# It4innovations/hyperqueue

Measured on AMD Instinct MI355X. Metric: tasks_assigned_per_sec, higher is better.
Workload: dtype u64

## Files before the change

hyperqueue_amd/csrc/debug_capi.cpp:

```cpp
#include "../../include/hqtick_debug.h"

#include "hb_order.h"
#include "milp.h"
#include "price_emul.h"

static thread_local int g_last_canonical = 0;
static thread_local long g_last_hull[2] = {0, 0};
extern "C" int hqtick_debug_milp_was_canonical(void) { return g_last_canonical; }
extern "C" void hqtick_debug_milp_last_hull(long *solves, long *nonpacking) {
    if (solves) *solves = g_last_hull[0];
    if (nonpacking) *nonpacking = g_last_hull[1];
}

extern "C" int hqtick_debug_milp_solve(int ncols, const double *obj, const uint8_t *col_kind, int nrows, const uint8_t *row_type,
                                       const double *rhs, const int *row_off, const int *row_col, const double *row_coef,
                                       double time_limit_s, int canonical, double *x_out, double *obj_out, int *is_optimal,
                                       long *nodes_out) {
    hqmilp::Model m;
    m.obj.assign(obj, obj + ncols);
    m.kind.assign(col_kind, col_kind + ncols);
    m.rtype.assign(row_type, row_type + nrows);
    m.rhs.assign(rhs, rhs + nrows);
    m.roff.assign(row_off, row_off + nrows + 1);
    int nnz = nrows ? row_off[nrows] : 0;
    m.rcol.assign(row_col, row_col + nnz);
    m.rcoef.assign(row_coef, row_coef + nnz);
    hqmilp::Result r = hqmilp::solve(m, time_limit_s, canonical != 0);
    g_last_canonical = r.canonical ? 1 : 0;
    g_last_hull[0] = r.hull_solves; g_last_hull[1] = r.hull_solves_nonpacking;
    if (nodes_out) *nodes_out = r.nodes;
    if (!r.feasible) return 0;
    for (int j = 0; j < ncols; j++) x_out[j] = r.x[j];
    *obj_out = r.objective;
    *is_optimal = r.optimal ? 1 : 0;
    return 1;
}

extern "C" void hqtick_debug_map_order_u32(const uint32_t *keys, uint32_t n, uint32_t *out_pos) {
    std::vector<uint32_t> order;
    hqhb::insertion_order_u32(keys, n, order);
    for (uint32_t i = 0; i < n; i++) out_pos[i] = order[i];
}

extern "C" int hqtick_debug_milp_solve_priced(int ncols, const double *obj, const uint8_t *col_kind, const int32_t *col_group, int nrows, const uint8_t *row_type,
                                              const uint8_t *row_implied, const double *rhs, const int *row_off, const int *row_col, const double *row_coef,
                                              double time_limit_s, int use_sweeps, uint32_t min_cols, double *x_out, double *obj_out, int *is_optimal, double *stats_out) {
    hqmilp::Model m;
    m.obj.assign(obj, obj + ncols);
    m.kind.assign(col_kind, col_kind + ncols);
    m.rtype.assign(row_type, row_type + nrows);
    m.rhs.assign(rhs, rhs + nrows);
    m.roff.assign(row_off, row_off + nrows + 1);
    int nnz = nrows ? row_off[nrows] : 0;
    m.rcol.assign(row_col, row_col + nnz);
    m.rcoef.assign(row_coef, row_coef + nnz);
    if (col_group) m.col_group.assign(col_group, col_group + ncols);
    if (row_implied) m.row_implied.assign(row_implied, row_implied + nrows);
    hqprice::EmulatedSweeper emu;
    if (min_cols) emu.min_cols = min_cols;
    hqmilp::Result r = hqmilp::solve(m, time_limit_s, true, hqmilp::REFERENCE_MIP_REL_GAP, use_sweeps ? &emu : nullptr);
    g_last_canonical = r.canonical ? 1 : 0;
    g_last_hull[0] = r.hull_solves; g_last_hull[1] = r.hull_solves_nonpacking;
    if (stats_out) { stats_out[0] = r.price_sweeps; stats_out[1] = r.price_rounds; stats_out[2] = r.price_total_us; stats_out[3] = r.canonical ? 1.0 : 0.0; }
    if (!r.feasible) return 0;
    for (int j = 0; j < ncols; j++) x_out[j] = r.x[j];
    *obj_out = r.objective;
    *is_optimal = r.optimal ? 1 : 0;
    return 1;
}

static thread_local hqmilp::Probe g_block_run_probe;
extern "C" void hqtick_debug_set_block_runs(int on) {
    hqmilp::g_probe = on < 0 ? nullptr : &g_block_run_probe; hqmilp::set_block_runs(on);
    if (on >= 0) { g_block_run_probe.model = g_block_run_probe.tables = g_block_run_probe.runs = g_block_run_probe.covered = 0; }
}
extern "C" void hqtick_debug_corrupt_block_runs(int on) { g_block_run_probe.corrupt_runs = on != 0; }
extern "C" void hqtick_debug_last_coupled_digest(uint64_t out[4]) {
    out[0] = g_block_run_probe.model; out[1] = g_block_run_probe.tables; out[2] = g_block_run_probe.runs; out[3] = g_block_run_probe.covered;
}
```

hyperqueue_amd/csrc/price.cpp:

```cpp
#include "price.h"

#include <algorithm>
#include <chrono>
#include <cmath>
#include <cstdio>
#include <cstring>
#include <functional>
#include <map>
#include <numeric>

#include "lp_tab.h"
#include "milp.h"

namespace hqprice {
namespace {

using hqmilp::lp::BASIC;
using hqmilp::lp::INF;
using hqmilp::lp::LP_OPT;
using hqmilp::lp::Rows;
using hqmilp::lp::Tab;

constexpr int KMAX_HOST = 128;
constexpr int NMAX_BLOCK = 32, MMAX_BLOCK = 4;
constexpr double FIRST_PROPOSAL_SCALE = 1.0 / 16.0;
constexpr double GRID = 10000.0;
constexpr int MAX_ROUNDS = 6;
constexpr int BP_MAX_NODES = 600;
constexpr double BP_MAX_STEPS = 3.0e6;
constexpr double BP_MAX_WORK = 3.0e9;

double now_us() { return std::chrono::duration<double, std::micro>(std::chrono::steady_clock::now().time_since_epoch()).count(); }

struct CapRow { int flat; double rhs; std::vector<std::pair<int, double>> g; };

struct Prob {
    HostTables T;
    std::vector<int> flat_of, model_of;
    std::vector<int> gmodel;
    std::vector<double> gcost;
    int K = 0, G = 0;
    std::vector<double> h;
    std::vector<uint8_t> ge;
    std::vector<std::vector<std::pair<int, double>>> g_rows;
    std::vector<int> grp_of;
    int KG = 0;
    std::vector<int> g_off, g_col; std::vector<int32_t> g_coef;
    std::vector<int> gr_off, gr_row;
    size_t row_terms = 0;
    std::vector<CapRow> caps;
    std::vector<int32_t> base_cap;
    std::vector<int> block_of_flat;
    int n_runs = 0, run_blocks = 0;
};

inline double round_fast(double v) { return (double)(long long)(v + (v >= 0.0 ? 0.5 : -0.5)); }
long long gcd_ll(long long a, long long b) { while (b) { const long long t = a % b; a = b; b = t; } return a < 0 ? -a : a; }

void finish_groups(Prob &P, const std::vector<std::vector<std::pair<int, int32_t>>> &lhs) {
    HostTables &T = P.T;
    const int KG = P.KG;
    T.K = (uint32_t)KG;
    size_t tot = 0; for (auto &l : lhs) tot += l.size();
    P.g_off.assign((size_t)KG + 1, 0); P.g_col.resize(tot); P.g_coef.resize(tot);
    std::vector<uint32_t> gcnt(T.n_cols + 1, 0);
    {
        auto *gc = P.g_col.data(); auto *gk = P.g_coef.data(); uint32_t *cnt = gcnt.data() + 1; size_t pos = 0;
        for (int g = 0; g < KG; g++) {
            const std::pair<int, int32_t> *l = lhs[(size_t)g].data();
            for (size_t i = 0, e = lhs[(size_t)g].size(); i < e; i++) { gc[pos] = l[i].first; gk[pos] = l[i].second; cnt[l[i].first]++; pos++; }
            P.g_off[(size_t)g + 1] = (int)pos;
        }
    }
    T.col_woff.assign(T.n_cols + 1, 0);
    for (uint32_t f = 0; f < T.n_cols; f++) T.col_woff[f + 1] = T.col_woff[f] + gcnt[f + 1];
    T.w_row.resize(T.col_woff[T.n_cols]); T.w_coef.resize(T.col_woff[T.n_cols]);
    {
        std::vector<uint32_t> &cur = gcnt;
        for (uint32_t f = 0; f < T.n_cols; f++) cur[f] = T.col_woff[f];
        uint32_t *cp = cur.data(); uint16_t *wr = T.w_row.data(); auto *wc = T.w_coef.data();
        const auto *gc = P.g_col.data(); const auto *gk = P.g_coef.data();
        for (int g = 0; g < KG; g++) for (int e = P.g_off[g], e1 = P.g_off[g + 1]; e < e1; e++) { const uint32_t p = cp[gc[e]]++; wr[p] = (uint16_t)g; wc[p] = gk[e]; }
    }
    P.gr_off.assign((size_t)KG + 1, 0);
    for (int k = 0; k < P.K; k++) P.gr_off[P.grp_of[k] + 1]++;
    for (int g = 0; g < KG; g++) P.gr_off[g + 1] += P.gr_off[g];
    P.gr_row.resize(P.K);
    { std::vector<int> c2(P.gr_off.begin(), P.gr_off.end() - 1); for (int k = 0; k < P.K; k++) P.gr_row[c2[P.grp_of[k]]++] = k; }
}

const char *build(const Request &rq, Prob &P) {
    const int n = rq.n;
    if (!rq.col_group) return "no block hints";
    std::vector<int> gid; gid.reserve(n);
    int max_group = -1;
    for (int j = 0; j < n; j++) max_group = std::max(max_group, rq.col_group[j]);
    std::vector<int> block_of_group((size_t)max_group + 1, -1);
    std::vector<int> bsize;
    std::vector<int> blk(n, -1);
    for (int j = 0; j < n; j++) {
        const int g = rq.col_group[j];
        if (g < 0) { P.gmodel.push_back(j); continue; }
        if (block_of_group[g] < 0) { block_of_group[g] = (int)bsize.size(); bsize.push_back(0); }
        blk[j] = block_of_group[g];
        if (++bsize[blk[j]] > NMAX_BLOCK) return "block with more than 32 columns";
    }
    const int nb = (int)bsize.size();
    if (nb < 8) return "fewer than 8 blocks";
    P.G = (int)P.gmodel.size();
    for (int j : P.gmodel) {
        if (rq.ub[j] != 1.0) return "global column that is not 0/1";
        if (rq.c[j] < 0.0) return "global column with negative cost";
        P.gcost.push_back(rq.c[j]);
    }
    std::vector<int> gidx(n, -1);
    for (int g = 0; g < P.G; g++) gidx[P.gmodel[g]] = g;
    HostTables &T = P.T;
    T.n_blocks = (uint32_t)nb;
    T.blk_off.assign((size_t)nb + 1, 0);
    for (int b = 0; b < nb; b++) T.blk_off[b + 1] = T.blk_off[b] + (uint32_t)bsize[b];
    T.n_cols = T.blk_off[nb];
    P.flat_of.assign(n, -1); P.model_of.assign(T.n_cols, -1); P.block_of_flat.assign(T.n_cols, -1);
    {
        std::vector<uint32_t> cur(T.blk_off.begin(), T.blk_off.end() - 1);
        for (int j = 0; j < n; j++) if (blk[j] >= 0) { const int f = (int)cur[blk[j]]++; P.flat_of[j] = f; P.model_of[f] = j; P.block_of_flat[f] = blk[j]; }
    }
    T.col_cost.assign(T.n_cols, 0.0); T.col_a.assign((size_t)T.n_cols * MMAX_BLOCK, 0.0); T.col_cap.assign(T.n_cols, 0);
    T.blk_m.assign(nb, 0); T.blk_cap.assign((size_t)nb * MMAX_BLOCK, 0.0);
    for (uint32_t f = 0; f < T.n_cols; f++) {
        const int j = P.model_of[f];
        if (rq.c[j] < 0.0) return "negative cost";
        if (!(rq.ub[j] <= 65535.0)) return "column bound above 65535";
        T.col_cost[f] = rq.c[j];
        T.col_cap[f] = (int32_t)std::floor(rq.ub[j] + 1e-9);
    }
    struct WideTmp { double h; uint8_t ge; std::vector<std::pair<int, int32_t>> cols; std::vector<std::pair<int, double>> g; };
    std::vector<WideTmp> wide;
    std::vector<std::pair<int, long long>> ai;
    for (int i = 0; i < rq.m; i++) {
        const int a = rq.roff[i], e = rq.roff[i + 1];
        if (a == e) continue;
        const double sc = rq.row_scale[i];
        int b0 = -2; bool multi = false, has_g = false, nonneg = true;
        int n_bcols = 0;
        for (int k = a; k < e; k++) {
            const int j = rq.rcol[k];
            if (rq.rcoef[k] < 0.0) nonneg = false;
            if (blk[j] < 0) { has_g = true; continue; }
            n_bcols++;
            if (b0 == -2) b0 = blk[j]; else if (blk[j] != b0) multi = true;
        }
        const bool is_le = rq.rlo[i] <= -INF, is_ge = rq.rhi[i] >= INF;
        if (is_le && is_ge) continue;
        if (!multi && !has_g && b0 >= 0) {
            if (rq.row_implied && rq.row_implied[i]) continue;
            if (is_le && nonneg) {
                double amax = 0.0;
                for (int k = a; k < e; k++) amax += rq.rcoef[k] * rq.ub[rq.rcol[k]];
                if (amax <= rq.rhi[i] * (1.0 + 1e-12) + 1e-9) continue;
            }
            if (!is_le || !nonneg || rq.rhi[i] < 0.0) return "block row that is not a packing row";
            const int r = T.blk_m[b0];
            if (r >= MMAX_BLOCK) {
                if (rq.trace) { fprintf(stderr, "[price] 5th row of block %d: hi %.6f scale %.6f:", b0, rq.rhi[i], sc); for (int k = a; k < e; k++) fprintf(stderr, " %.6f*x%d(ub %.0f)", rq.rcoef[k] * sc, rq.rcol[k], rq.ub[rq.rcol[k]]); fprintf(stderr, "\n"); }
                return "block with more than 4 rows";
            }
            long long g = 0; bool ok = true;
            ai.clear();
            for (int k = a; k < e && ok; k++) {
                const double v = rq.rcoef[k] * sc * GRID, rv = std::round(v);
                if (rv < 1.0 || std::fabs(v - rv) > 1e-6 * std::max(1.0, rv) || rv >= 4.0e15) ok = false;
                else { ai.push_back({P.flat_of[rq.rcol[k]], (long long)rv}); g = gcd_ll(g, (long long)rv); }
            }
            if (!ok) return "block row off the ResourceAmount grid";
            const double capv = rq.rhi[i] * sc * GRID;
            if (capv >= 4.0e15) return "block row capacity too large";
            const long long capi = (long long)std::floor(capv + 1e-6);
            if (g < 1) g = 1;
            for (auto &t : ai) T.col_a[(size_t)t.first * MMAX_BLOCK + r] += (double)(t.second / g);
            T.blk_cap[(size_t)b0 * MMAX_BLOCK + r] = (double)(capi / g);
            T.blk_m[b0] = (uint8_t)(r + 1);
            continue;
        }
        if (!is_le && !is_ge) return "equality or range row across blocks";
        if (is_le && nonneg) {
            double amax = 0.0;
            for (int k = a; k < e; k++) amax += rq.rcoef[k] * rq.ub[rq.rcol[k]];
            if (amax <= rq.rhi[i] * (1.0 + 1e-12) + 1e-9) continue;
        }
        if (is_ge && nonneg && rq.rlo[i] <= 1e-12) continue;
        if (!multi && has_g && n_bcols >= 1 && is_le && nonneg) {
            if (n_bcols != 1) return "conditional bound over several columns of a block";
            CapRow cr; cr.flat = -1; cr.rhs = 0.0;
            double cx = 0.0;
            for (int k = a; k < e; k++) if (blk[rq.rcol[k]] >= 0) { cr.flat = P.flat_of[rq.rcol[k]]; cx = rq.rcoef[k]; }
            if (!(cx > 0.0)) return "conditional bound with a zero coefficient";
            cr.rhs = rq.rhi[i] / cx;
            for (int k = a; k < e; k++) if (blk[rq.rcol[k]] < 0) cr.g.push_back({gidx[rq.rcol[k]], rq.rcoef[k] / cx});
            P.caps.push_back(std::move(cr));
            continue;
        }
        if (n_bcols == 0) return "row over global columns only";
        WideTmp w; w.ge = is_ge ? 1 : 0;
        w.cols.reserve((size_t)(e - a));
        const double sign = is_le ? 1.0 : -1.0;
        w.h = sign * (is_le ? rq.rhi[i] : rq.rlo[i]) * sc;
        for (int k = a; k < e; k++) {
            const int j = rq.rcol[k];
            const double v = sign * rq.rcoef[k] * sc;
            if (blk[j] < 0) { w.g.push_back({gidx[j], v}); continue; }
            const double rv = std::round(v);
            if (std::fabs(v - rv) > 1e-7 * std::max(1.0, std::fabs(rv)) || std::fabs(rv) > 1.0e9) return "wide row with a non-integer coefficient";
            if (rv != 0.0) w.cols.push_back({P.flat_of[j], (int32_t)rv});
        }
        wide.push_back(std::move(w));
        if ((int)wide.size() > 1024) return "more than 1024 wide rows";
    }
    for (int b = 0; b < nb; b++) if (T.blk_m[b] == 0) {
        double total = 0.0;
        for (uint32_t f = T.blk_off[b]; f < T.blk_off[b + 1]; f++) { T.col_a[(size_t)f * MMAX_BLOCK] = 1.0; total += (double)T.col_cap[f]; }
        T.blk_cap[(size_t)b * MMAX_BLOCK] = total;
        T.blk_m[b] = 1;
    }
    P.K = (int)wide.size();
    if (P.K == 0) return "no wide row";
    P.h.resize(P.K); P.ge.resize(P.K); P.g_rows.assign(P.G, {});
    std::vector<uint64_t> sig(P.K);
    for (int k = 0; k < P.K; k++) {
        P.h[k] = wide[k].h; P.ge[k] = wide[k].ge;
        uint64_t hsh = 1469598103934665603ull;
        for (auto &t : wide[k].cols) { hsh = (hsh ^ (uint64_t)(uint32_t)t.first) * 1099511628211ull; hsh = (hsh ^ (uint64_t)(uint32_t)t.second) * 1099511628211ull; }
        sig[k] = hsh; P.row_terms += wide[k].cols.size();
        for (auto &t : wide[k].g) P.g_rows[t.first].push_back({k, t.second});
    }
    P.grp_of.assign(P.K, -1);
    std::vector<int> rep;
    for (int k = 0; k < P.K; k++) {
        int g = -1;
        for (size_t i = 0; i < rep.size() && g < 0; i++) if (sig[rep[i]] == sig[k] && wide[rep[i]].cols == wide[k].cols) g = (int)i;
        if (g < 0) { g = (int)rep.size(); rep.push_back(k); }
        P.grp_of[k] = g;
    }
    P.KG = (int)rep.size();
    if (P.KG > KMAX_HOST) return "more than 128 distinct wide left-hand sides";
    std::vector<std::vector<std::pair<int, int32_t>>> lhs((size_t)P.KG);
    for (int g = 0; g < P.KG; g++) lhs[(size_t)g] = std::move(wide[rep[g]].cols);
    finish_groups(P, lhs);
    P.base_cap = T.col_cap;
    return nullptr;
}

struct Cut {
    double cx = 0, bnd = 0; std::vector<long long> act; std::vector<double> pi;
    std::vector<uint16_t> x; bool fetched = false; std::vector<std::pair<uint32_t, int32_t>> lo;
    std::vector<double> pcx; std::vector<long long> pact;
};

struct BPNode { std::vector<int8_t> flag; std::vector<std::pair<uint32_t, int32_t>> lo, hi; double bound = INF; int depth = 0; };

struct Solver {
    const Request &rq; Sweeper &sw; Prob P;
    std::vector<Cut> cuts;
    double relaxed_bound = INF;
    std::vector<double> relaxed_pi;
    double theta_scale = 1.0;
    std::vector<double> pmax;
    bool failed = false;
    size_t cut_lo = 0;
    double work = 0.0;
    double sweep_steps = 0.0; int budget_sweeps = 0;
    int max_sweeps = 256;
    std::vector<std::pair<uint32_t, int32_t>> node_lo, node_caps; double node_cl = 0.0; std::vector<double> node_Al; bool at_root = true;
    bool base_caps = true;
    Solver(const Request &r, Sweeper &s) : rq(r), sw(s) {}

    bool evaluate_launch(const std::vector<double> &pi) {
        if ((int)cuts.size() >= max_sweeps) return false;
        std::vector<double> pig(P.KG, 0.0);
        for (int k = 0; k < P.K; k++) pig[P.grp_of[k]] += pi[k];
        const double t0 = now_us();
        sw.pending_k = (uint32_t)P.KG;
        if (!sw.sweep_launch(pig.data())) { failed = true; return false; }
        sw.stat_sweep_us += now_us() - t0;
        return true;
    }
    int evaluate(const std::vector<double> &pi, bool launched = false) {
        if ((int)cuts.size() >= max_sweeps) return -1;
        SweepTotals tot;
        const double t0 = now_us();
        if (launched) { if (!sw.sweep_finish(tot)) { failed = true; return -1; } }
        else {
            std::vector<double> pig(P.KG, 0.0);
            for (int k = 0; k < P.K; k++) pig[P.grp_of[k]] += pi[k];
            if (!sw.sweep(pig.data(), tot)) { failed = true; return -1; }
        }
        sw.stat_sweep_us += now_us() - t0; sw.stat_sweeps++;
        if (!sw.merges_clock() && now_us() * 1e-6 > sw.guard_s) sw.time_up = true;
        sweep_steps += 64.0 + (double)tot.max_steps;
        if (tot.n_budget > std::max<uint32_t>(4, P.T.n_blocks / 64)) budget_sweeps++;
        Cut c; c.cx = tot.cx; c.bnd = tot.bnd; c.pi = pi;
        c.act.resize(P.K);
        for (int k = 0; k < P.K; k++) c.act[k] = tot.act[P.grp_of[k]];
        if (node_lo.empty() && tot.part_cx.size() == (size_t)PARTS && tot.part_act.size() == (size_t)PARTS * P.KG) {
            c.pcx = tot.part_cx; c.pact.resize((size_t)PARTS * P.K);
            for (int p = 0; p < PARTS; p++) for (int k = 0; k < P.K; k++) c.pact[(size_t)p * P.K + k] = tot.part_act[(size_t)p * P.KG + P.grp_of[k]];
        }
        if (!node_lo.empty()) {
            c.lo = node_lo; c.cx += node_cl; c.bnd += node_cl;
            for (int k = 0; k < P.K; k++) { c.act[k] += (long long)std::llround(node_Al[k]); c.bnd -= pi[k] * node_Al[k]; }
        }
        cuts.push_back(std::move(c));
        double L = cuts.back().bnd;
        for (int k = 0; k < P.K; k++) L += pi[k] * P.h[k];
        for (int g = 0; g < P.G; g++) { double r = P.gcost[g]; for (auto &t : P.g_rows[g]) r -= pi[t.first] * t.second; if (r > 0.0) L += r; }
        if (base_caps && at_root && L < relaxed_bound) { relaxed_bound = L; relaxed_pi = pi; }
        return (int)cuts.size() - 1;
    }
    double fixed_value(const Cut &c, const std::vector<double> &hB, double cB) const {
        double L = c.bnd + cB;
        for (int k = 0; k < P.K; k++) L += c.pi[k] * hB[k];
        return L;
    }

    bool aggregate_prices(const std::vector<double> &hB, const std::vector<int> &lk, std::vector<double> &pi) {
        const HostTables &T = P.T;
        static const int chunks_env = getenv("HQPRICE_AGG_CHUNKS") ? atoi(getenv("HQPRICE_AGG_CHUNKS")) : 0;
        uint32_t widest = 1;
        for (uint32_t b = 0; b < T.n_blocks; b++) widest = std::max(widest, T.blk_off[b + 1] - T.blk_off[b]);
        const int agg_chunks = chunks_env > 0 ? chunks_env : std::min(64, std::max(PARTS, (int)(256u / widest)));
        const uint32_t nb = T.n_blocks, per = (nb + (uint32_t)agg_chunks - 1) / (uint32_t)agg_chunks;
        const int NP = (int)((nb + per - 1) / per), KL = (int)lk.size();
        if (NP < 2 || KL == 0) return false;
        static const uint64_t min_cols_env = getenv("HQPRICE_AGG_MINCOLS") ? (uint64_t)atoll(getenv("HQPRICE_AGG_MINCOLS")) : 32768;
        if ((uint64_t)T.n_cols < min_cols_env) return false;
        if (P.G != 0) return false;
        std::vector<uint32_t> pb0(NP), pcnt(NP), pnc(NP), voff(NP + 1, 0);
        for (int p = 0; p < NP; p++) {
            const uint32_t b0 = (uint32_t)p * per, b1 = std::min(nb, b0 + per);
            pb0[p] = b0; pcnt[p] = b1 - b0; pnc[p] = T.blk_off[b0 + 1] - T.blk_off[b0];
            const uint32_t c0 = T.blk_off[b0], nc = pnc[p];
            for (uint32_t b = b0 + 1; b < b1; b++) {
                const uint32_t c = T.blk_off[b];
                if (T.blk_off[b + 1] - c != nc || T.blk_m[b] != T.blk_m[b0]) return false;
                if (memcmp(&T.blk_cap[(size_t)b * MMAX_BLOCK], &T.blk_cap[(size_t)b0 * MMAX_BLOCK], sizeof(double) * MMAX_BLOCK) != 0) return false;
                if (memcmp(&T.col_a[(size_t)c * MMAX_BLOCK], &T.col_a[(size_t)c0 * MMAX_BLOCK], sizeof(double) * MMAX_BLOCK * nc) != 0) return false;
                if (memcmp(&T.col_cap[c], &T.col_cap[c0], sizeof(int32_t) * nc) != 0) return false;
                for (uint32_t q = 0; q < nc; q++) {
                    const uint32_t e0 = T.col_woff[c0 + q], e1 = T.col_woff[c0 + q + 1], f0 = T.col_woff[c + q];
                    if (T.col_woff[c + q + 1] - f0 != e1 - e0) return false;
                    if (e1 > e0 && (memcmp(&T.w_row[f0], &T.w_row[e0], sizeof(uint16_t) * (e1 - e0)) != 0 || memcmp(&T.w_coef[f0], &T.w_coef[e0], sizeof(int32_t) * (e1 - e0)) != 0)) return false;
                }
            }
            voff[p + 1] = voff[p] + nc;
        }
        const int nv = (int)voff[NP];
        if (nv == 0 || nv > 8192) return false;
        Rows A; A.n = nv;
        std::vector<double> ac(nv), alb(nv, 0.0), aub(nv);
        std::vector<std::pair<int, double>> terms;
        for (int p = 0; p < NP; p++) {
            const uint32_t c0 = T.blk_off[pb0[p]], nc = pnc[p];
            for (uint32_t q = 0; q < nc; q++) {
                double sum = 0.0;
                for (uint32_t b = 0; b < pcnt[p]; b++) sum += T.col_cost[T.blk_off[pb0[p] + b] + q];
                ac[voff[p] + q] = sum / (double)pcnt[p] / theta_scale;
                aub[voff[p] + q] = (double)pcnt[p] * (double)T.col_cap[c0 + q];
            }
            for (int r = 0; r < (int)T.blk_m[pb0[p]]; r++) {
                terms.clear(); double sc = 0.0;
                for (uint32_t q = 0; q < nc; q++) { const double a = T.col_a[(size_t)(c0 + q) * MMAX_BLOCK + r]; if (a != 0.0) { terms.push_back({(int)(voff[p] + q), a}); sc = std::max(sc, std::fabs(a)); } }
                if (terms.empty()) continue;
                for (auto &t : terms) t.second /= sc;
                A.add(terms, -INF, (double)pcnt[p] * T.blk_cap[(size_t)pb0[p] * MMAX_BLOCK + r] / sc);
            }
        }
        const int first_wide = A.m;
        std::vector<double> wscale(KL, 1.0);
        for (int i = 0; i < KL; i++) {
            const int g = P.grp_of[lk[i]];
            terms.clear(); double sc = 0.0;
            for (int p = 0; p < NP; p++) {
                const uint32_t c0 = T.blk_off[pb0[p]];
                for (uint32_t q = 0; q < pnc[p]; q++) for (uint32_t e = T.col_woff[c0 + q]; e < T.col_woff[c0 + q + 1]; e++) if ((int)T.w_row[e] == g) { terms.push_back({(int)(voff[p] + q), (double)T.w_coef[e]}); sc = std::max(sc, std::fabs((double)T.w_coef[e])); }
            }
            if (terms.empty()) { A.add({{0, 0.0}}, -INF, INF); continue; }
            for (auto &t : terms) t.second /= sc;
            wscale[i] = sc;
            A.add(terms, -INF, hB[lk[i]] / sc);
        }
        Tab at; at.init(&A, ac, alb, aub);
        if (at.solve(20000) != LP_OPT) return false;
        work += at.ops;
        pi.assign(P.K, 0.0);
        bool any = false;
        for (int i = 0; i < KL; i++) {
            const int a = at.where[first_wide + i];
            if (a < 0 || at.st[A.n + a] == BASIC) continue;
            double y = std::fabs(at.d[A.n + a]) / wscale[i] * theta_scale;
            if (!(y > 0.0)) continue;
            pi[lk[i]] = std::min(y, pmax[lk[i]]);
            any = true;
        }
        return any;
    }

    std::function<bool(const std::vector<double> &, double)> probe;
    struct Settled { bool valid = false; std::vector<double> hB, lambda, pi; double cB = 0.0, bound = 0.0; size_t n_cuts = 0, cut_lo = 0; } settled;
    bool kelley(const std::vector<double> &hB, double cB, double cutoff, double tol, std::vector<double> &lambda, std::vector<double> &pi_out, double *bound_out, bool no_sweeps = false) {
        if (!no_sweeps && settled.valid) {
            settled.valid = false;
            if (settled.n_cuts == cuts.size() && settled.cut_lo == cut_lo && settled.cB == cB && settled.hB == hB) {
                if (settled.bound < cutoff) return false;
                lambda = std::move(settled.lambda); pi_out = std::move(settled.pi); *bound_out = settled.bound;
                return true;
            }
        }
        const int K = P.K;
        const uint32_t per = (P.T.n_blocks + PARTS - 1) / PARTS;
        const int NP = (int)((P.T.n_blocks + per - 1) / per);
        std::vector<int> lk; lk.reserve(P.KG);
        for (int g = 0; g < P.KG; g++) {
            int best = -1;
            for (int q = P.gr_off[g]; q < P.gr_off[g + 1]; q++) { const int k = P.gr_row[q]; if (best < 0 || hB[k] < hB[best]) best = k; }
            if (best >= 0) lk.push_back(best);
        }
        std::sort(lk.begin(), lk.end());
        const int KL = (int)lk.size();
        Rows M; M.n = KL + NP;
        std::vector<double> mc(KL + NP), mlb(KL + NP, 0.0), mub(KL + NP);
        for (int i = 0; i < KL; i++) { mc[i] = -hB[lk[i]] / theta_scale; mub[i] = pmax[lk[i]]; }
        for (int p = 0; p < NP; p++) { mc[KL + p] = -1.0; mub[KL + p] = 4.0; }
        std::vector<double> cut_scale;
        std::vector<std::pair<int, double>> terms;
        size_t in_master = cut_lo;
        auto push_cuts = [&](Tab *mt) {
            for (; in_master < cuts.size(); in_master++) {
                const Cut &c = cuts[in_master];
                for (int p = 0; p < NP; p++) {
                    terms.clear(); double sc = 1.0;
                    for (int i = 0; i < KL; i++) { const long long a = c.pact[(size_t)p * K + lk[i]]; if (a != 0) { const double v = (double)a / theta_scale; terms.push_back({i, v}); sc = std::max(sc, std::fabs(v)); } }
                    terms.push_back({KL + p, 1.0});
                    for (auto &t : terms) t.second /= sc;
                    M.add(terms, c.pcx[p] / theta_scale / sc, INF);
                    cut_scale.push_back(sc);
                    if (mt) mt->where.push_back(-1);
                }
            }
        };
        for (size_t k = cut_lo; k < cuts.size(); k++) if (cuts[k].pcx.empty()) { if (rq.trace) fprintf(stderr, "[price] master: cut %zu without part sums\n", k); return false; }
        push_cuts(nullptr);
        Tab mt; mt.init(&M, mc, mlb, mub);
        double ub_best = INF; std::vector<double> pi_best(K, 0.0);
        for (size_t k = cut_lo; k < cuts.size(); k++) { const double L = fixed_value(cuts[k], hB, cB); if (L < ub_best) { ub_best = L; pi_best = cuts[k].pi; } }
        std::vector<double> pi(K, 0.0), pi_prev_master;
        double lb_master = -INF, lp_us = 0.0;
        bool converged = false; int probes = 0;
        auto multipliers = [&](std::vector<double> &lambda) {
            lambda.assign(cuts.size() * PARTS, 0.0);
            std::vector<double> lsum(NP, 0.0);
            for (size_t r = 0; r / NP + cut_lo < cuts.size() && r < (size_t)M.m; r++) {
                const int a = mt.where[r];
                if (a < 0 || mt.st[M.n + a] == BASIC) continue;
                const size_t k = r / NP + cut_lo; const int p = (int)(r % NP);
                const double v = std::fabs(mt.d[M.n + a]) / cut_scale[r];
                lambda[k * PARTS + p] = v; lsum[p] += v;
            }
            for (int p = 0; p < NP; p++) if (!(lsum[p] > 0.0)) {
                size_t bk = cut_lo; double bv = -INF;
                for (size_t k = cut_lo; k < cuts.size(); k++) {
                    double v = cuts[k].pcx[p];
                    for (int i = 0; i < KL; i++) v -= mt.x[i] * (double)cuts[k].pact[(size_t)p * K + lk[i]];
                    if (v > bv) { bv = v; bk = k; }
                }
                lambda[bk * PARTS + p] = 1.0; lsum[p] = 1.0;
            }
            for (size_t k = cut_lo; k < cuts.size(); k++) for (int p = 0; p < NP; p++) lambda[k * PARTS + p] /= lsum[p];
        };
        for (int it = 0; it < 200; it++) {
            { const double tl0 = now_us(); const int st = mt.solve(200000); lp_us += now_us() - tl0; if (st != LP_OPT) { if (rq.trace) fprintf(stderr, "[price] master LP status %d at iteration %d (%d cuts)\n", st, it, M.m); return false; } }
            lb_master = -mt.objective() * theta_scale + cB;
            if (ub_best < cutoff) { if (rq.trace) fprintf(stderr, "[price] configuration bounded by %.9f, below the incumbent %.9f\n", ub_best, cutoff); return false; }
            if (ub_best - lb_master <= tol * std::fabs(ub_best)) { converged = true; break; }
            if (no_sweeps) return false;
            if (probe && probes < 3 && it >= 1 && ub_best - lb_master <= 0.1 * std::fabs(ub_best)) {
                probes++;
                std::vector<double> lam, colact(K, 0.0);
                multipliers(lam);
                for (size_t k = cut_lo; k < cuts.size(); k++) for (int p = 0; p < NP; p++) {
                    const double l = lam[k * PARTS + p];
                    if (l == 0.0) continue;
                    const long long *pa = &cuts[k].pact[(size_t)p * K];
                    for (int r = 0; r < K; r++) colact[r] += l * (double)pa[r];
                }
                auto keep = std::move(probe); probe = nullptr;
                const bool go = keep(colact, lb_master);
                probe = std::move(keep);
                if (go) return false;
            }
            bool same = !pi_prev_master.empty();
            for (int i = 0; i < KL && same; i++) same = std::fabs(mt.x[i] - pi_prev_master[i]) <= 1e-15 + 1e-12 * std::fabs(mt.x[i]);
            pi_prev_master.assign(mt.x.begin(), mt.x.begin() + KL);
            const double alpha = (it < 3 || same) ? 0.0 : 0.3;
            for (int k = 0; k < K; k++) pi[k] = alpha * pi_best[k];
            for (int i = 0; i < KL; i++) pi[lk[i]] += (1.0 - alpha) * mt.x[i];
            if (it == 0 && cut_lo == 0 && cuts.size() == 1) {
                std::vector<double> pa;
                static const bool agg_on = !(getenv("HQPRICE_AGG_START") && atoi(getenv("HQPRICE_AGG_START")) == 0);
                if (agg_on && aggregate_prices(hB, lk, pa)) { pi = pa; if (rq.trace) fprintf(stderr, "[price]   first proposal: the duals of the model aggregated over chunks of blocks\n"); }
                else for (int k = 0; k < K; k++) pi[k] *= FIRST_PROPOSAL_SCALE;
            }
            const int ci = evaluate(pi);
            if (ci < 0) break;
            if (sw.time_up) { if (rq.trace) fprintf(stderr, "[price] 70 %% of the time limit gone inside the master loop\n"); return false; }
            if (budget_sweeps >= 8) { if (rq.trace) fprintf(stderr, "[price] blocks keep running out of their search budget (%d sweeps): not a model for the sweeps\n", budget_sweeps); return false; }
            const double L = fixed_value(cuts[ci], hB, cB);
            if (L < ub_best) { ub_best = L; pi_best = pi; }
            push_cuts(&mt);
        }
        if (!converged) {
            if (mt.solve(200000) != LP_OPT) return false;
            lb_master = -mt.objective() * theta_scale + cB;
            if (ub_best - lb_master > 1e-3 * std::fabs(ub_best)) { if (rq.trace) fprintf(stderr, "[price] master not converged: %.9f vs %.9f\n", ub_best, lb_master); return false; }
        }
        multipliers(lambda);
        if (rq.trace) fprintf(stderr, "[price]   master: %d priced rows + %d parts, %d cut rows, %ld pivots, %.1f us inside the LP (%d active rows)\n", KL, NP, M.m, mt.iters, lp_us, mt.ma);
        pi_out.assign(K, 0.0);
        for (int i = 0; i < KL; i++) pi_out[lk[i]] = mt.x[i];
        *bound_out = ub_best;
        if (no_sweeps) { settled.valid = true; settled.hB = hB; settled.cB = cB; settled.lambda = lambda; settled.pi = pi_out; settled.bound = ub_best; settled.n_cuts = cuts.size(); settled.cut_lo = cut_lo; }
        return true;
    }

    bool fetch_patterns() {
        size_t first = cuts.size();
        for (size_t k = 0; k < cuts.size(); k++) if (!cuts[k].fetched) { first = k; break; }
        if (first == cuts.size()) return true;
        const uint32_t count = (uint32_t)(cuts.size() - first);
        const uint16_t *pat = sw.patterns((uint32_t)first, count);
        if (!pat) { failed = true; return false; }
        const uint32_t nc = P.T.n_cols;
        for (uint32_t i = 0; i < count; i++) {
            Cut &c = cuts[first + i];
            if (c.fetched) continue;
            c.x.assign(pat + (size_t)i * nc, pat + (size_t)(i + 1) * nc);
            for (auto &l : c.lo) c.x[l.first] = (uint16_t)(c.x[l.first] + l.second);
            c.fetched = true;
        }
        return true;
    }

    std::vector<uint16_t> round_patterns(const std::vector<double> &lambda, const std::vector<double> &pi, const std::vector<double> &hB,
                                         const std::vector<char> *usable = nullptr, const std::vector<int32_t> *lo_of = nullptr, int variant = 0) {
        const int K = P.K; const HostTables &T = P.T;
        const uint32_t S = (uint32_t)cuts.size();
        const double t_r0 = now_us();
        if (!fetch_patterns()) return {};
        auto pat_of = [&](int k) { return cuts[(size_t)k].x.data(); };
        const uint32_t per = (T.n_blocks + PARTS - 1) / PARTS;
        auto lam = [&](int k, uint32_t p) { return lambda[(size_t)k * PARTS + p]; };
        std::vector<int> active;
        for (uint32_t k = 0; k < S; k++) {
            if (usable && !(*usable)[k]) continue;
            bool any = false; for (uint32_t p = 0; p < (uint32_t)PARTS && !any; p++) any = lam((int)k, p) > 1e-9;
            if (any) active.push_back((int)k);
        }
        if (active.empty()) return {};
        const int Q = (int)active.size();
        std::vector<double> lpact(K, 0.0), wgt(K);
        for (int k : active) {
            const Cut &c = cuts[k];
            if (c.pact.empty()) { for (int r = 0; r < K; r++) lpact[r] += lam(k, 0) * (double)c.act[r]; continue; }
            for (uint32_t p = 0; p < (uint32_t)PARTS; p++) { const double l = lam(k, p); if (l > 0.0) for (int r = 0; r < K; r++) lpact[r] += l * (double)c.pact[(size_t)p * P.K + r]; }
        }
        for (int r = 0; r < K; r++) {
            const bool tight = pi[r] > 1e-12 || hB[r] - lpact[r] <= 1e-6 * std::max(1.0, std::fabs(hB[r]));
            wgt[r] = (tight ? 1.0 : 0.02) / std::max(1.0, std::fabs(hB[r]));
        }
        auto block_act = [&](uint32_t b, const uint16_t *x, std::vector<double> &out) {
            double ga[KMAX_HOST];
            for (int g = 0; g < P.KG; g++) ga[g] = 0.0;
            for (uint32_t f = T.blk_off[b]; f < T.blk_off[b + 1]; f++) { const uint16_t xv = x[f]; if (!xv) continue; for (uint32_t e = T.col_woff[f]; e < T.col_woff[f + 1]; e++) ga[T.w_row[e]] += (double)T.w_coef[e] * (double)xv; }
            for (int r = 0; r < K; r++) out[r] = ga[P.grp_of[r]];
        };
        std::vector<uint16_t> x(T.n_cols, 0);
        std::vector<double> cum(K, 0.0);
        std::vector<int> chosen(T.n_blocks, 0);
        {
            const int KG = P.KG;
            std::vector<double> wg(KG, 0.0), cumg(KG, 0.0), tgtg(KG, 0.0), candg((size_t)Q * KG);
            for (int r = 0; r < K; r++) wg[P.grp_of[r]] += wgt[r];
            std::vector<char> on(Q); std::vector<const double *> cgp(Q, nullptr);
            for (uint32_t bi = 0; bi < T.n_blocks; bi++) {
                const uint32_t b = variant == 1 ? T.n_blocks - 1 - bi : bi;
                const uint32_t part = b / per;
                int first = -1; bool all_same = true;
                const size_t blk_bytes = (size_t)(T.blk_off[b + 1] - T.blk_off[b]) * 2;
                for (int q = 0; q < Q; q++) {
                    const double l = lam(active[q], part);
                    on[q] = l > 1e-9;
                    if (!on[q]) continue;
                    const uint16_t *px = pat_of(active[q]);
                    if (first >= 0 && memcmp(px + T.blk_off[b], pat_of(active[first]) + T.blk_off[b], blk_bytes) == 0) cgp[q] = cgp[first];
                    else {
                        if (first < 0) first = q; else all_same = false;
                        double *cg = &candg[(size_t)q * KG];
                        for (int g = 0; g < KG; g++) cg[g] = 0.0;
                        for (uint32_t f = T.blk_off[b]; f < T.blk_off[b + 1]; f++) { const uint16_t xv = px[f]; if (!xv) continue; for (uint32_t e = T.col_woff[f]; e < T.col_woff[f + 1]; e++) cg[T.w_row[e]] += (double)T.w_coef[e] * (double)xv; }
                        cgp[q] = cg;
                    }
                    const double *cg = cgp[q];
                    for (int g = 0; g < KG; g++) tgtg[g] += l * cg[g];
                }
                int bq = -1; double be = INF;
                if (all_same) bq = first;
                else for (int q = 0; q < Q; q++) {
                    if (!on[q]) continue;
                    const double *cg = cgp[q];
                    double e = 0.0;
                    for (int g = 0; g < KG; g++) e += std::fabs(cumg[g] + cg[g] - tgtg[g]) * wg[g];
                    if (e < be - 1e-15) { be = e; bq = q; }
                }
                if (bq < 0) return {};
                const double *cb = cgp[bq];
                for (int g = 0; g < KG; g++) cumg[g] += cb[g];
                chosen[b] = active[bq];
                memcpy(&x[T.blk_off[b]], pat_of(active[bq]) + T.blk_off[b], (size_t)(T.blk_off[b + 1] - T.blk_off[b]) * 2);
            }
            for (int r = 0; r < K; r++) cum[r] = cumg[P.grp_of[r]];
        }
        if (rq.trace) fprintf(stderr, "[price]   rounding: diffusion done at %.3f us, %d active cuts\n", now_us() - t_r0, Q);
        auto ge_short = [&](const std::vector<double> &c) { double s = 0.0; for (int r = 0; r < K; r++) if (P.ge[r] && c[r] > hB[r] + 1e-9) s += c[r] - hB[r]; return s; };
        if (ge_short(cum) > 0.0) {
            std::vector<int> pool = active;
            for (int k = (int)S - 1; k >= 0 && (int)pool.size() < Q + 12; k--) if ((!usable || (*usable)[k]) && std::find(pool.begin(), pool.end(), k) == pool.end()) pool.push_back(k);
            std::vector<double> a0(K), a1(K), c2(K);
            double cmax = 0.0; for (double c : T.col_cost) cmax = std::max(cmax, c);
            struct Cand { double score; uint32_t b; int k; };
            std::vector<Cand> cl; std::vector<double> colshort, coltight;
            auto evaluate_switch = [&](uint32_t b, int k, double v0, double &score) {
                const uint16_t *px = pat_of(k);
                block_act(b, px, a1);
                double gain = 0.0, newviol = 0.0;
                for (int r = 0; r < K; r++) {
                    if (a0[r] == a1[r]) continue;
                    const double c = cum[r] - a0[r] + a1[r];
                    if (P.ge[r]) gain += std::max(0.0, cum[r] - hB[r]) - std::max(0.0, c - hB[r]);
                    else newviol += std::max(0.0, c - hB[r]) - std::max(0.0, cum[r] - hB[r]);
                }
                if (!(gain > 1e-9)) return false;
                double v1 = 0.0; for (uint32_t f = T.blk_off[b]; f < T.blk_off[b + 1]; f++) v1 += T.col_cost[f] * (double)px[f];
                score = gain * 10.0 * cmax - (v0 - v1) - std::max(0.0, newviol) * cmax;
                return true;
            };
            auto value_of = [&](uint32_t b) { double v = 0.0; for (uint32_t f = T.blk_off[b]; f < T.blk_off[b + 1]; f++) v += T.col_cost[f] * (double)x[f]; return v; };
            for (int pass = 0; pass < 64 && ge_short(cum) > 0.0; pass++) {
                const double base = ge_short(cum);
                cl.clear();
                std::vector<int> short_in(P.KG, 0);
                for (int r = 0; r < K; r++) if (P.ge[r] && cum[r] > hB[r] + 1e-9) short_in[P.grp_of[r]]++;
                std::vector<int> tight_in(P.KG, 0);
                double spare = 0.0;
                for (int r = 0; r < K; r++) if (P.ge[r] && cum[r] <= hB[r] + 1e-9 && hB[r] - cum[r] <= 2.0 + 1e-9) { tight_in[P.grp_of[r]]++; spare += std::max(0.0, hB[r] - cum[r]); }
                colshort.assign(T.n_cols, 0.0); coltight.assign(T.n_cols, 0.0);
                for (uint32_t f = 0; f < T.n_cols; f++) for (uint32_t e = T.col_woff[f]; e < T.col_woff[f + 1]; e++) {
                    const int ns = short_in[T.w_row[e]], nt = tight_in[T.w_row[e]];
                    if (ns) colshort[f] += (double)ns * (double)T.w_coef[e];
                    if (nt) coltight[f] += (double)nt * (double)T.w_coef[e];
                }
                for (uint32_t b = 0; b < T.n_blocks; b++) {
                    for (int k : pool) {
                        if (k == chosen[b]) continue;
                        const uint16_t *px = pat_of(k);
                        double gain = 0.0, dv = 0.0, dmg = 0.0; bool differs = false;
                        for (uint32_t f = T.blk_off[b]; f < T.blk_off[b + 1]; f++) {
                            const int d = (int)px[f] - (int)x[f];
                            if (!d) continue;
                            differs = true; dv += T.col_cost[f] * (double)d;
                            gain -= colshort[f] * (double)d;
                            dmg += coltight[f] * (double)d;
                        }
                        if (!differs || !(gain - std::max(0.0, dmg - spare) > 1e-9)) continue;
                        cl.push_back({std::min(gain, base) * 10.0 * cmax + dv, b, k});
                    }
                }
                if (rq.trace) fprintf(stderr, "[price]     pass %d: short by %.1f, %zu candidate switches, at %.3f us\n", pass, base, cl.size(), now_us() - t_r0);
                if (cl.empty()) break;
                const size_t top = std::min<size_t>(cl.size(), 512);
                std::partial_sort(cl.begin(), cl.begin() + (long)top, cl.end(), [](const Cand &p, const Cand &q) { return p.score > q.score || (p.score == q.score && (p.b < q.b || (p.b == q.b && p.k < q.k))); });
                cl.resize(top);
                std::vector<char> moved(T.n_blocks, 0);
                for (const Cand &cd : cl) {
                    if (!(ge_short(cum) > 0.0)) break;
                    if (moved[cd.b]) continue;
                    {
                        const uint16_t *px = pat_of(cd.k); double gain = 0.0;
                        for (uint32_t f = T.blk_off[cd.b]; f < T.blk_off[cd.b + 1]; f++) {
                            const int d = (int)px[f] - (int)x[f];
                            if (d) for (uint32_t e = T.col_woff[f]; e < T.col_woff[f + 1]; e++) { const int g = T.w_row[e]; for (int q = P.gr_off[g]; q < P.gr_off[g + 1]; q++) { const int r = P.gr_row[q]; if (P.ge[r] && cum[r] > hB[r] + 1e-9) gain -= (double)T.w_coef[e] * (double)d; } }
                        }
                        if (!(gain > 1e-9)) continue;
                    }
                    block_act(cd.b, pat_of(chosen[cd.b]), a0);
                    double score;
                    if (!evaluate_switch(cd.b, cd.k, value_of(cd.b), score)) continue;
                    for (int r = 0; r < K; r++) cum[r] += a1[r] - a0[r];
                    chosen[cd.b] = cd.k; moved[cd.b] = 1;
                    memcpy(&x[T.blk_off[cd.b]], pat_of(cd.k) + T.blk_off[cd.b], (size_t)(T.blk_off[cd.b + 1] - T.blk_off[cd.b]) * 2);
                }
                if (ge_short(cum) >= base - 1e-9) break;
            }
            if (ge_short(cum) > 0.0) return {};
        }
        if (rq.trace) fprintf(stderr, "[price]   rounding: >= repair done at %.3f us\n", now_us() - t_r0);
        for (int r = 0; r < K; r++) {
            if (cum[r] <= hB[r] + 1e-9) continue;
            std::vector<int> cols;
            const int gr = P.grp_of[r];
            for (int k = P.g_off[gr]; k < P.g_off[gr + 1]; k++) if (P.g_coef[k] > 0 && x[P.g_col[k]] > 0) cols.push_back(k);
            std::sort(cols.begin(), cols.end(), [&](int a, int b) { const double ca = T.col_cost[P.g_col[a]] / P.g_coef[a], cb = T.col_cost[P.g_col[b]] / P.g_coef[b]; return ca < cb || (ca == cb && a > b); });
            for (int k : cols) {
                const int f = P.g_col[k];
                while (x[f] > (lo_of ? (uint16_t)(*lo_of)[f] : 0) && cum[r] > hB[r] + 1e-9) {
                    bool ok = true;
                    for (uint32_t e = T.col_woff[f]; e < T.col_woff[f + 1] && ok; e++) if (T.w_coef[e] < 0) { const int g = T.w_row[e]; for (int q = P.gr_off[g]; q < P.gr_off[g + 1] && ok; q++) if (cum[P.gr_row[q]] - (double)T.w_coef[e] > hB[P.gr_row[q]] + 1e-9) ok = false; }
                    if (!ok) break;
                    x[f]--;
                    for (uint32_t e = T.col_woff[f]; e < T.col_woff[f + 1]; e++) { const int g = T.w_row[e]; for (int q = P.gr_off[g]; q < P.gr_off[g + 1]; q++) cum[P.gr_row[q]] -= (double)T.w_coef[e]; }
                }
                if (cum[r] <= hB[r] + 1e-9) break;
            }
            if (cum[r] > hB[r] + 1e-9) return {};
        }
        return x;
    }

    struct NodeLP { double bound = INF; bool pruned = false; std::vector<double> lambda, pi, bfrac; };

    bool apply_node(const BPNode &nd, std::vector<int32_t> &lo_arr, std::vector<int32_t> &hi_arr) {
        const HostTables &T = P.T;
        lo_arr.assign(T.n_cols, 0); hi_arr = P.base_cap;
        for (auto &l : nd.lo) lo_arr[l.first] = std::max(lo_arr[l.first], l.second);
        for (auto &h : nd.hi) hi_arr[h.first] = std::min(hi_arr[h.first], h.second);
        node_caps.clear();
        for (const CapRow &cr : P.caps) {
            double r = cr.rhs; bool all_fixed = true;
            for (auto &t : cr.g) { if (nd.flag[t.first] < 0) { all_fixed = false; break; } r -= t.second * (double)nd.flag[t.first]; }
            if (!all_fixed) continue;
            const double c = std::floor(r + 1e-9);
            const int32_t cap = c < 0.0 ? 0 : (c > 65535.0 ? 65535 : (int32_t)c);
            if (cap < hi_arr[cr.flat]) { hi_arr[cr.flat] = cap; node_caps.push_back({(uint32_t)cr.flat, cap}); }
        }
        std::vector<int32_t> caps(T.n_cols); std::vector<double> bcap(T.blk_cap);
        node_lo.clear(); node_cl = 0.0; node_Al.assign(P.K, 0.0);
        for (uint32_t f = 0; f < T.n_cols; f++) {
            if (hi_arr[f] < lo_arr[f]) return false;
            caps[f] = hi_arr[f] - lo_arr[f];
            const int32_t l = lo_arr[f];
            if (l <= 0) continue;
            node_lo.push_back({f, l}); node_cl += T.col_cost[f] * (double)l;
            for (uint32_t e = T.col_woff[f]; e < T.col_woff[f + 1]; e++) { const int g = T.w_row[e]; for (int q = P.gr_off[g]; q < P.gr_off[g + 1]; q++) node_Al[P.gr_row[q]] += (double)T.w_coef[e] * (double)l; }
            const int b = P.block_of_flat[f];
            for (int r = 0; r < MMAX_BLOCK; r++) bcap[(size_t)b * MMAX_BLOCK + r] -= T.col_a[(size_t)f * MMAX_BLOCK + r] * (double)l;
        }
        for (double v : bcap) if (v < 0.0) return false;
        if (!sw.set_caps(caps.data()) || !sw.set_block_caps(bcap.data())) { failed = true; return false; }
        at_root = nd.lo.empty() && nd.hi.empty() && node_caps.empty();
        return true;
    }

    void node_master(const BPNode &nd, double cutoff, double tol, NodeLP &out, std::vector<char> &usable) {
        const int K = P.K, G = P.G;
        out = NodeLP(); out.bound = nd.bound;
        if (!fetch_patterns()) return;
        usable.assign(cuts.size(), 1);
        for (size_t k = 0; k < cuts.size(); k++) {
            const std::vector<uint16_t> &x = cuts[k].x;
            for (auto &l : nd.lo) if ((int32_t)x[l.first] < l.second) { usable[k] = 0; break; }
            if (usable[k]) for (auto &h : nd.hi) if ((int32_t)x[h.first] > h.second) { usable[k] = 0; break; }
            if (usable[k]) for (auto &h : node_caps) if ((int32_t)x[h.first] > h.second) { usable[k] = 0; break; }
        }
        std::vector<double> hN(P.h); double cN = 0.0;
        std::vector<int> freeg;
        for (int g = 0; g < G; g++) {
            if (nd.flag[g] < 0) { freeg.push_back(g); continue; }
            cN += P.gcost[g] * (double)nd.flag[g];
            for (auto &t : P.g_rows[g]) hN[t.first] -= t.second * (double)nd.flag[g];
        }
        const int F = (int)freeg.size();
        Rows M; M.n = K + 1 + F;
        std::vector<double> mc(M.n), mlb(M.n, 0.0), mub(M.n);
        for (int k = 0; k < K; k++) { mc[k] = -hN[k] / theta_scale; mub[k] = pmax[k]; }
        mc[K] = -1.0; mub[K] = 4.0;
        for (int i = 0; i < F; i++) { mc[K + 1 + i] = -1.0; mub[K + 1 + i] = 4.0; }
        std::vector<std::pair<int, double>> terms;
        std::vector<double> row_scale; std::vector<int> row_cut;
        for (int i = 0; i < F; i++) {
            const int g = freeg[i];
            terms.clear(); double sc = 1.0;
            for (auto &t : P.g_rows[g]) { const double v = t.second / theta_scale; terms.push_back({t.first, v}); sc = std::max(sc, std::fabs(v)); }
            terms.push_back({K + 1 + i, 1.0});
            for (auto &t : terms) t.second /= sc;
            M.add(terms, P.gcost[g] / theta_scale / sc, INF);
            row_scale.push_back(sc); row_cut.push_back(-1);
        }
        Tab mt;
        auto add_cut = [&](size_t k, bool live) {
            const Cut &c = cuts[k];
            terms.clear(); double sc = 1.0;
            for (int r = 0; r < K; r++) if (c.act[r] != 0) { const double v = (double)c.act[r] / theta_scale; terms.push_back({r, v}); sc = std::max(sc, std::fabs(v)); }
            terms.push_back({K, 1.0});
            for (auto &t : terms) t.second /= sc;
            M.add(terms, c.cx / theta_scale / sc, INF);
            row_scale.push_back(sc); row_cut.push_back((int)k);
            if (live) mt.where.push_back(-1);
        };
        for (size_t k = 0; k < cuts.size(); k++) if (usable[k]) add_cut(k, false);
        mt.init(&M, mc, mlb, mub);
        auto node_value = [&](const Cut &c) {
            double L = c.bnd + cN;
            for (int k = 0; k < K; k++) L += c.pi[k] * hN[k];
            for (int g : freeg) { double r = P.gcost[g]; for (auto &t : P.g_rows[g]) r -= c.pi[t.first] * t.second; if (r > 0.0) L += r; }
            return L;
        };
        std::vector<double> pi(K), pi_best, prev;
        bool ok = false;
        for (int it = 0; it < 80; it++) {
            ok = false;
            if (mt.solve(200000) != LP_OPT) break;
            ok = true;
            const double lbm = -mt.objective() * theta_scale + cN;
            if (out.bound <= cutoff) { out.pruned = true; break; }
            if (out.bound - lbm <= tol * std::fabs(out.bound)) break;
            bool same = !prev.empty();
            for (int k = 0; k < K && same; k++) same = std::fabs(mt.x[k] - prev[k]) <= 1e-15 + 1e-12 * std::fabs(mt.x[k]);
            prev.assign(mt.x.begin(), mt.x.begin() + K);
            const double alpha = (it < 2 || same || pi_best.empty()) ? 0.0 : 0.3;
            for (int k = 0; k < K; k++) pi[k] = (alpha > 0.0 ? alpha * pi_best[k] : 0.0) + (1.0 - alpha) * mt.x[k];
            const int ci = evaluate(pi);
            if (ci < 0) { ok = false; break; }
            usable.push_back(1);
            const double L = node_value(cuts[ci]);
            if (L < out.bound) { out.bound = L; pi_best = pi; }
            add_cut((size_t)ci, true);
        }
        work += mt.ops;
        if (!ok || out.pruned) return;
        out.lambda.assign(cuts.size(), 0.0); out.bfrac.assign(G, 0.0);
        double lsum = 0.0;
        for (int r = 0; r < M.m; r++) {
            const int a = mt.where[r];
            if (a < 0 || mt.st[M.n + a] == BASIC) continue;
            const double v = std::fabs(mt.d[M.n + a]) / row_scale[r];
            if (row_cut[r] >= 0) { out.lambda[row_cut[r]] = v; lsum += v; } else out.bfrac[freeg[r]] = std::min(1.0, v);
        }
        for (int g = 0; g < G; g++) if (nd.flag[g] >= 0) out.bfrac[g] = (double)nd.flag[g];
        if (lsum > 0.0) for (double &l : out.lambda) l /= lsum; else out.lambda.clear();
        out.pi.assign(mt.x.begin(), mt.x.begin() + K);
    }
};

}

namespace {
Answer run_solver(Solver &S, const double tp0) {
    Answer ans;
    const Request &rq = S.rq; Sweeper &sw = S.sw;
    auto tmark = [&](const char *what) { if (rq.trace) fprintf(stderr, "[price] %s at %.3f ms (sweeps so far %.3f ms)\n", what, (now_us() - tp0) / 1e3, sw.stat_sweep_us / 1e3); };
    tmark("model flattened");
    if (rq.trace) fprintf(stderr, "[price]   %d equal-block runs took %d of %u blocks from their first one\n", S.P.n_runs, S.P.run_blocks, S.P.T.n_blocks);
    Prob &P = S.P;
    if (rq.trace) fprintf(stderr, "[price] %u blocks, %u block columns, %d wide rows with %d distinct left-hand sides (%zu / %zu terms), %d flags, %zu conditional bounds\n", P.T.n_blocks, P.T.n_cols, P.K, P.KG, P.row_terms, P.T.w_row.size(), P.G, P.caps.size());
    const int K = P.K, G = P.G;
    sw.stat_sweeps = 0; sw.stat_sweep_us = 0;
    sw.guard_s = rq.deadline_s - 0.3 * rq.time_limit_s; sw.time_up = false;
    S.max_sweeps = (int)std::min<size_t>(4096, std::max<size_t>(256, ((size_t)64 << 20) / ((size_t)P.T.n_cols * 2 + 1)));
    if (!sw.begin(P.T, (uint32_t)S.max_sweeps)) { ans.why = "sweeper refused the model"; return ans; }
    struct Ender { Sweeper &s; ~Ender() { s.end(); } } ender{sw};
    tmark("tables handed to the sweeper");
    std::vector<double> pi0(K, 0.0);
    if (!S.evaluate_launch(pi0)) { ans.why = "sweep failed"; return ans; }
    S.pmax.assign(K, 0.0);
    {
        double cmax = 0.0; for (double c : P.T.col_cost) cmax = std::max(cmax, c);
        std::vector<double> gp(P.KG, 0.0);
        for (int g = 0; g < P.KG; g++) {
            double p = 0.0; bool neg = false; int32_t amin = INT32_MAX;
            for (int t = P.g_off[g]; t < P.g_off[g + 1]; t++) {
                const int32_t a = P.g_coef[t];
                if (a > 0) p = std::max(p, P.T.col_cost[P.g_col[t]] / (double)a); else { neg = true; amin = std::min(amin, -a); }
            }
            if (neg) p = std::max(p, 64.0 * cmax / (double)std::max<int32_t>(1, amin));
            gp[g] = p;
        }
        for (int k = 0; k < K; k++) S.pmax[k] = gp[P.grp_of[k]];
    }
    tmark("price caps done");
    if (S.evaluate(pi0, true) < 0) { ans.why = "sweep failed"; return ans; }
    tmark("first sweep (prices 0) done");
    S.theta_scale = std::max(S.cuts[0].bnd, 1e-9);
    ans.ran = true;
    double best_value = rq.incumbent ? rq.incumbent_value : -INF;
    std::vector<double> hB(K);
    std::vector<int32_t> caps(P.base_cap);
    std::vector<double> final_pi;
    std::vector<std::vector<double>> tried;
    auto was_tried = [&](const std::vector<double> &B) { for (auto &t : tried) if (t == B) return true; return false; };
    auto certified = [&]() { return best_value > -INF && S.relaxed_bound <= best_value + rq.rel_gap * std::fabs(best_value); };
    std::vector<double> jump_to;
    auto try_config = [&](const std::vector<double> &B, std::vector<double> &x) -> double {
        tried.push_back(B);
        if (!sw.merges_clock() && now_us() * 1e-6 > sw.guard_s) sw.time_up = true;
        if (sw.time_up) return -INF;
        ans.rounds++;
        double cB = 0.0;
        for (int k = 0; k < K; k++) hB[k] = P.h[k];
        for (int g = 0; g < G; g++) { cB += P.gcost[g] * B[g]; for (auto &t : P.g_rows[g]) hB[t.first] -= t.second * B[g]; }
        if (!P.caps.empty()) {
            caps = P.base_cap;
            for (const CapRow &cr : P.caps) { double r = cr.rhs; for (auto &t : cr.g) r -= t.second * B[t.first]; const double c = std::floor(r + 1e-9); if (c < (double)caps[cr.flat]) caps[cr.flat] = c < 0.0 ? 0 : (int32_t)c; }
            if (!sw.set_caps(caps.data())) { S.failed = true; return -INF; }
            S.base_caps = false; S.cut_lo = S.cuts.size();
            if (S.evaluate(pi0) < 0) return -INF;
        }
        std::vector<double> lambda, pi;
        double bound_B = INF;
        const double cutoff = best_value > -INF ? best_value * (1.0 - 1e-12) : -INF;
        const double tol = std::max(1e-6, rq.rel_gap / 50.0);
        jump_to.clear();
        S.probe = nullptr;
        if (G > 0 && P.caps.empty()) S.probe = [&](const std::vector<double> &colact, double lb_here) -> bool {
            std::vector<double> Bp = B, act = colact;
            for (int g = 0; g < G; g++) if (Bp[g] == 1.0) for (auto &t : P.g_rows[g]) act[t.first] += t.second;
            bool dropped = false;
            for (int g = 0; g < G; g++) {
                if (Bp[g] != 1.0 || P.gcost[g] != 0.0) continue;
                bool ok = true;
                for (auto &t : P.g_rows[g]) if (act[t.first] - t.second > P.h[t.first] + 1e-7 * (1.0 + std::fabs(P.h[t.first]))) ok = false;
                if (!ok) continue;
                Bp[g] = 0.0; dropped = true;
                for (auto &t : P.g_rows[g]) act[t.first] -= t.second;
            }
            if (!dropped || was_tried(Bp)) return false;
            std::vector<double> hBp(K); double cBp = 0.0;
            for (int k = 0; k < K; k++) hBp[k] = P.h[k];
            for (int g = 0; g < G; g++) { cBp += P.gcost[g] * Bp[g]; for (auto &t : P.g_rows[g]) hBp[t.first] -= t.second * Bp[g]; }
            std::vector<double> lam2, pi2; double b2 = INF;
            if (!S.kelley(hBp, cBp, -INF, tol, lam2, pi2, &b2, true) || b2 < lb_here) { S.settled.valid = false; return false; }
            if (rq.trace) fprintf(stderr, "[price] configuration %u left for the one its fractional point names: converged on the %zu cuts at hand, bound %.9f\n", ans.rounds, S.cuts.size(), b2);
            jump_to = Bp;
            return true;
        };
        const bool conv = S.kelley(hB, cB, cutoff, tol, lambda, pi, &bound_B);
        S.probe = nullptr;
        if (!conv) return -INF;
        tmark("master converged");
        final_pi = pi;
        std::vector<uint16_t> xf = S.round_patterns(lambda, pi, hB);
        tmark("patterns rounded");
        if (xf.empty()) return -INF;
        x.assign(rq.n, 0.0);
        for (uint32_t f = 0; f < P.T.n_cols; f++) x[P.model_of[f]] = (double)xf[f];
        for (int g = 0; g < G; g++) x[P.gmodel[g]] = B[g];
        double value = 0.0;
        if (!rq.polish || !rq.polish(x, value)) return -INF;
        tmark("polished");
        if (rq.trace) fprintf(stderr, "[price] configuration %u: %zu sweeps so far, bound with these flags %.9f, point %.9f, model bound %.9f\n", ans.rounds, S.cuts.size(), bound_B, value, S.relaxed_bound);
        if (value > best_value) { best_value = value; ans.x = x; ans.x_value = value; }
        if (bound_B > best_value * (1.0 + rq.rel_gap)) {
            std::vector<uint16_t> xr = S.round_patterns(lambda, pi, hB, nullptr, nullptr, 1);
            if (!xr.empty()) {
                std::vector<double> x2(rq.n, 0.0);
                for (uint32_t f = 0; f < P.T.n_cols; f++) x2[P.model_of[f]] = (double)xr[f];
                for (int g = 0; g < G; g++) x2[P.gmodel[g]] = B[g];
                double v2 = 0.0;
                if (rq.polish(x2, v2)) {
                    if (rq.trace) fprintf(stderr, "[price] configuration %u, blocks in reverse order: point %.9f\n", ans.rounds, v2);
                    if (v2 > value) { value = v2; x = x2; }
                    if (v2 > best_value) { best_value = v2; ans.x = x2; ans.x_value = v2; }
                }
            }
        }
        return value;
    };
    auto drop_flags = [&](std::vector<double> &B, const std::vector<double> &x) {
        bool dropped = false;
        std::vector<double> act(K, 0.0);
        {
            std::vector<double> ga(P.KG, 0.0);
            for (int g = 0; g < P.KG; g++) for (int t = P.g_off[g]; t < P.g_off[g + 1]; t++) ga[g] += (double)P.g_coef[t] * x[P.model_of[P.g_col[t]]];
            for (int k = 0; k < K; k++) act[k] += ga[P.grp_of[k]];
        }
        for (int g = 0; g < G; g++) for (auto &t : P.g_rows[g]) act[t.first] += t.second * x[P.gmodel[g]];
        for (int g = 0; g < G; g++) {
            if (B[g] != 1.0 || P.gcost[g] != 0.0 || x[P.gmodel[g]] != 1.0) continue;
            bool ok = true;
            for (auto &t : P.g_rows[g]) if (act[t.first] - t.second > P.h[t.first] + 1e-7 * (1.0 + std::fabs(P.h[t.first]))) ok = false;
            if (!ok) continue;
            B[g] = 0.0; dropped = true;
            for (auto &t : P.g_rows[g]) act[t.first] -= t.second;
        }
        return dropped;
    };
    auto descend = [&](std::vector<double> B) {
        for (int round = 0; round < MAX_ROUNDS && !S.failed && !was_tried(B); round++) {
            std::vector<double> x;
            const double v = try_config(B, x);
            if (!jump_to.empty()) { B = jump_to; jump_to.clear(); continue; }
            if (v == -INF) break;
            if (certified()) break;
            if (!drop_flags(B, x)) break;
        }
    };
    if (rq.incumbent && G > 0) {
        std::vector<double> B(G);
        for (int g = 0; g < G; g++) B[g] = rq.incumbent[P.gmodel[g]] > 0.5 ? 1.0 : 0.0;
        descend(B);
    }
    if (ans.x.empty() && !S.failed) descend(std::vector<double>(G, 1.0));
    if (S.failed) { ans.ran = false; ans.why = "sweep failed"; ans.x.clear(); return ans; }
    std::vector<double> Blp;
    if (G > 0 && best_value > -INF && !certified()) {
        if (!S.base_caps) {
            if (!sw.set_caps(P.base_cap.data())) { ans.ran = false; ans.why = "sweep failed"; ans.x.clear(); return ans; }
            S.base_caps = true; S.cut_lo = S.cuts.size();
            if (S.evaluate(pi0) < 0) { ans.ran = false; ans.why = "sweep failed"; ans.x.clear(); return ans; }
        }
        Rows M; M.n = K + 1 + G;
        std::vector<double> mc(M.n), mlb(M.n, 0.0), mub(M.n);
        for (int k = 0; k < K; k++) { mc[k] = -P.h[k] / S.theta_scale; mub[k] = S.pmax[k]; }
        mc[K] = -1.0; mub[K] = 4.0;
        for (int g = 0; g < G; g++) { mc[K + 1 + g] = -1.0; mub[K + 1 + g] = 4.0; }
        std::vector<std::pair<int, double>> terms;
        for (int g = 0; g < G; g++) {
            terms.clear(); double sc = 1.0;
            for (auto &t : P.g_rows[g]) { const double v = t.second / S.theta_scale; terms.push_back({t.first, v}); sc = std::max(sc, std::fabs(v)); }
            terms.push_back({K + 1 + g, 1.0});
            for (auto &t : terms) t.second /= sc;
            M.add(terms, P.gcost[g] / S.theta_scale / sc, INF);
        }
        size_t in_master = S.cut_lo;
        Tab mt;
        auto push_cuts = [&](bool live) {
            for (; in_master < S.cuts.size(); in_master++) {
                const Cut &c = S.cuts[in_master];
                terms.clear(); double sc = 1.0;
                for (int k = 0; k < K; k++) if (c.act[k] != 0) { const double v = (double)c.act[k] / S.theta_scale; terms.push_back({k, v}); sc = std::max(sc, std::fabs(v)); }
                terms.push_back({K, 1.0});
                for (auto &t : terms) t.second /= sc;
                M.add(terms, c.cx / S.theta_scale / sc, INF);
                if (live) mt.where.push_back(-1);
            }
        };
        push_cuts(false);
        mt.init(&M, mc, mlb, mub);
        std::vector<double> pi(K), pi_best = S.relaxed_pi.empty() ? std::vector<double>(K, 0.0) : S.relaxed_pi, prev;
        bool master_ok = false;
        for (int it = 0; it < 120; it++) {
            master_ok = false;
            if (mt.solve(200000) != LP_OPT) break;
            master_ok = true;
            const double lb_master = -mt.objective() * S.theta_scale;
            if (S.relaxed_bound <= best_value + rq.rel_gap * std::fabs(best_value)) break;
            if (S.relaxed_bound - lb_master <= 1e-6 * std::fabs(S.relaxed_bound)) break;
            bool same = !prev.empty();
            for (int k = 0; k < K && same; k++) same = std::fabs(mt.x[k] - prev[k]) <= 1e-15 + 1e-12 * std::fabs(mt.x[k]);
            prev.assign(mt.x.begin(), mt.x.begin() + K);
            const double alpha = (it < 2 || same) ? 0.0 : 0.3;
            for (int k = 0; k < K; k++) pi[k] = alpha * pi_best[k] + (1.0 - alpha) * mt.x[k];
            const double before = S.relaxed_bound;
            if (S.evaluate(pi) < 0) break;
            if (S.relaxed_bound < before) pi_best = pi;
            push_cuts(true);
        }
        if (S.failed) { ans.ran = false; ans.why = "sweep failed"; ans.x.clear(); return ans; }
        if (master_ok || mt.solve(200000) == LP_OPT) {
            Blp.assign(G, 0.0);
            for (int g = 0; g < G; g++) { const int ar = mt.where[g]; if (ar >= 0 && mt.st[M.n + ar] != BASIC) { double sc = 1.0; for (auto &t : P.g_rows[g]) sc = std::max(sc, std::fabs(t.second / S.theta_scale)); Blp[g] = std::min(1.0, std::fabs(mt.d[M.n + ar]) / sc); } }
        }
    }
    if (!Blp.empty() && !certified() && P.caps.empty()) {
        std::vector<double> B(G);
        for (int g = 0; g < G; g++) B[g] = (Blp[g] > 0.5 || P.gcost[g] > 0.0) ? 1.0 : 0.0;
        descend(B);
        for (int trial = 0; trial < 12 && !certified() && !S.failed && !ans.x.empty(); trial++) {
            std::vector<double> cur(G);
            for (int g = 0; g < G; g++) cur[g] = ans.x[P.gmodel[g]];
            int pick = -1; double pv = INF;
            for (int g = 0; g < G; g++) {
                if (cur[g] != 1.0 || P.gcost[g] != 0.0) continue;
                std::vector<double> t = cur; t[g] = 0.0;
                if (was_tried(t)) continue;
                if (Blp[g] < pv) { pv = Blp[g]; pick = g; }
            }
            if (pick < 0) break;
            cur[pick] = 0.0;
            descend(cur);
        }
        if (S.failed) { ans.ran = false; ans.why = "sweep failed"; ans.x.clear(); return ans; }
    }
    double bp_bound = INF;
    if (best_value > -INF && !certified() && !S.failed && P.T.n_cols <= 131072 && S.budget_sweeps < 8) {
        S.base_caps = true;
        int col_nodes = 0;
        auto closes = [&](double bound) { return bound <= best_value + rq.rel_gap * std::fabs(best_value); };
        std::vector<BPNode> stack;
        { BPNode root; root.flag.assign(G, -1); root.bound = S.relaxed_bound; stack.push_back(std::move(root)); }
        double closed_max = -INF;
        int nodes = 0;
        std::vector<int32_t> lo_arr, hi_arr; std::vector<char> usable;
        while (!stack.empty() && nodes < BP_MAX_NODES && (int)S.cuts.size() + 8 < S.max_sweeps && S.work < BP_MAX_WORK * rq.time_limit_s && S.sweep_steps < BP_MAX_STEPS * rq.time_limit_s &&
               !sw.time_up && !S.failed) {
            BPNode nd = std::move(stack.back()); stack.pop_back();
            if (!sw.merges_clock() && now_us() * 1e-6 > sw.guard_s) { sw.time_up = true; stack.push_back(std::move(nd)); break; }
            if (closes(nd.bound)) { closed_max = std::max(closed_max, nd.bound); continue; }
            nodes++;
            if (!S.apply_node(nd, lo_arr, hi_arr)) { if (S.failed) break; continue; }
            Solver::NodeLP lp;
            S.node_master(nd, best_value, std::max(2e-6, rq.rel_gap / 20.0), lp, usable);
            if (S.failed) break;
            if (lp.pruned || closes(lp.bound)) { closed_max = std::max(closed_max, std::min(lp.bound, nd.bound)); continue; }
            if (lp.lambda.empty()) { stack.push_back(std::move(nd)); break; }
            nd.bound = std::min(nd.bound, lp.bound);
            int bg = -1; double bd = 1e-6;
            for (int g = 0; g < G; g++) if (nd.flag[g] < 0) { const double d = std::min(lp.bfrac[g], 1.0 - lp.bfrac[g]); if (d > bd) { bd = d; bg = g; } }
            if (bg < 0) {
                std::vector<double> Bn(G), hBn(P.h);
                for (int g = 0; g < G; g++) { Bn[g] = lp.bfrac[g] > 0.5 ? 1.0 : 0.0; for (auto &t : P.g_rows[g]) hBn[t.first] -= t.second * Bn[g]; }
                std::vector<double> lam_parts(lp.lambda.size() * PARTS);
                for (size_t k = 0; k < lp.lambda.size(); k++) for (int p = 0; p < PARTS; p++) lam_parts[k * PARTS + p] = lp.lambda[k];
                std::vector<uint16_t> xf = S.round_patterns(lam_parts, lp.pi, hBn, &usable, &lo_arr);
                if (!xf.empty()) {
                    std::vector<double> x(rq.n, 0.0);
                    for (uint32_t f = 0; f < P.T.n_cols; f++) x[P.model_of[f]] = (double)xf[f];
                    for (int g = 0; g < G; g++) x[P.gmodel[g]] = Bn[g];
                    double value = 0.0;
                    if (rq.polish && rq.polish(x, value) && value > best_value) { best_value = value; ans.x = x; ans.x_value = value; }
                }
                if (closes(nd.bound)) { closed_max = std::max(closed_max, nd.bound); continue; }
            }
            BPNode a = nd, b = nd; a.depth = b.depth = nd.depth + 1;
            if (bg >= 0) {
                const int8_t first = lp.bfrac[bg] > 0.5 ? 1 : 0;
                a.flag[bg] = first; b.flag[bg] = (int8_t)(1 - first);
            } else {
                if (++col_nodes > 48) { stack.push_back(std::move(nd)); break; }
                int bf = -1; double bs = 1e-7, bv = 0.0;
                std::vector<double> xl(P.T.n_cols, 0.0);
                for (size_t k = 0; k < S.cuts.size(); k++) { const double l = k < lp.lambda.size() ? lp.lambda[k] : 0.0; if (l <= 0.0 || !usable[k]) continue; const uint16_t *px = S.cuts[k].x.data(); for (uint32_t f = 0; f < P.T.n_cols; f++) xl[f] += l * (double)px[f]; }
                for (uint32_t f = 0; f < P.T.n_cols; f++) { const double fr = xl[f] - std::floor(xl[f]); const double sc = std::min(fr, 1.0 - fr) * (P.T.col_cost[f] + 1e-9); if (std::min(fr, 1.0 - fr) > 1e-6 && sc > bs) { bs = sc; bf = (int)f; bv = xl[f]; } }
                if (bf < 0) { closed_max = std::max(closed_max, nd.bound); continue; }
                const int32_t fl = (int32_t)std::floor(bv);
                BPNode dn = nd, up = nd; dn.depth = up.depth = nd.depth + 1;
                dn.hi.push_back({(uint32_t)bf, fl}); up.lo.push_back({(uint32_t)bf, fl + 1});
                if (bv - fl < 0.5) { a = std::move(dn); b = std::move(up); } else { a = std::move(up); b = std::move(dn); }
            }
            stack.push_back(std::move(b)); stack.push_back(std::move(a));
        }
        bp_bound = closed_max;
        for (const BPNode &nd : stack) bp_bound = std::max(bp_bound, nd.bound);
        if (rq.trace) fprintf(stderr, "[price] branch and price: %d nodes, %zu left open, %zu sweeps in all, bound %.9f, incumbent %.9f\n", nodes, stack.size(), S.cuts.size(), bp_bound, best_value);
        S.node_lo.clear(); S.at_root = true;
        if (S.failed) { ans.ran = false; ans.why = "sweep failed"; ans.x.clear(); return ans; }
    }
    ans.bound = std::min(S.relaxed_bound, bp_bound > -INF ? bp_bound : INF);
    ans.sweeps = (uint32_t)sw.stat_sweeps;
    const bool closed = best_value > -INF && ans.bound <= best_value + rq.rel_gap * std::fabs(best_value);
    if (!final_pi.empty() && !closed) {
        ans.block_of.assign(rq.n, -1); ans.rcost.assign(rq.n, 0.0);
        std::vector<std::pair<int, double>> rows;
        for (uint32_t f = 0; f < P.T.n_cols; f++) {
            const int j = P.model_of[f];
            ans.block_of[j] = P.block_of_flat[f];
            double r = P.T.col_cost[f];
            rows.clear();
            for (uint32_t e = P.T.col_woff[f]; e < P.T.col_woff[f + 1]; e++) { const int g = P.T.w_row[e]; for (int q = P.gr_off[g]; q < P.gr_off[g + 1]; q++) rows.push_back({P.gr_row[q], (double)P.T.w_coef[e]}); }
            std::sort(rows.begin(), rows.end());
            for (auto &t : rows) r -= final_pi[t.first] * t.second;
            ans.rcost[j] = r;
        }
    }
    return ans;
}
}

namespace {

thread_local bool g_check_hints = false; thread_local int g_hint_mismatches = 0;
const char *flatten_model(const ModelView &mv, Prob &P, std::vector<double> &ub, std::vector<double> &c, double &cmax) {
    const int n = mv.n, m = mv.m;
    if (!mv.col_group || !mv.row_lhs || !mv.row_lhs_len) return "no structure hints";
    int max_group = -1;
    for (int j = 0; j < n; j++) max_group = std::max(max_group, mv.col_group[j]);
    std::vector<int> block_of_group((size_t)max_group + 1, -1), bsize, blk(n, -1);
    for (int j = 0; j < n; j++) {
        const int g = mv.col_group[j];
        if (g < 0) { P.gmodel.push_back(j); continue; }
        if (block_of_group[g] < 0) { block_of_group[g] = (int)bsize.size(); bsize.push_back(0); }
        blk[j] = block_of_group[g];
        if (++bsize[blk[j]] > NMAX_BLOCK) return "block with more than 32 columns";
    }
    const int nb = (int)bsize.size();
    if (nb < 8) return "fewer than 8 blocks";
    cmax = 0.0;
    for (int j = 0; j < n; j++) cmax = std::max(cmax, std::fabs(mv.obj[j]));
    if (cmax == 0.0) cmax = 1.0;
    c.resize(n);
    for (int j = 0; j < n; j++) c[j] = mv.obj[j] / cmax;
    P.G = (int)P.gmodel.size();
    for (int j : P.gmodel) {
        if (mv.kind[j] != 1) return "global column that is not 0/1";
        if (c[j] < 0.0) return "global column with negative cost";
        P.gcost.push_back(c[j]);
    }
    std::vector<int> gidx(n, -1);
    for (int g = 0; g < P.G; g++) gidx[P.gmodel[g]] = g;
    const int n_lhs = mv.n_lists;
    for (int i = 0; i < m; i++) if (mv.row_lhs[i] >= n_lhs) return "bad structure hint";
    struct Fam { int first = -1, len = 0; bool has_neg = false, scanned = false; double rhs_min = INF;
                 int b0 = -2; bool multi = false, has_g = false, integral = true; int n_bcols = 0; double amax = 0.0; };
    std::vector<Fam> fam((size_t)n_lhs);
    ub.assign(n, INF);
    for (int j = 0; j < n; j++) if (mv.kind[j] == 1) ub[j] = 1.0;
    const bool hinted = mv.row_block && mv.col_ub;
    if (hinted) for (int j = 0; j < n; j++) if (mv.col_ub[j] != UINT32_MAX) ub[j] = std::min(ub[j], (double)mv.col_ub[j]);
    auto bound_terms = [&](int a, int e, double rhs) { for (int k = a; k < e; k++) if (mv.rcoef[k] > 0.0) { double &u = ub[mv.rcol[k]]; u = std::min(u, std::floor(rhs / mv.rcoef[k] + 1e-9)); } };
    for (int l = 0; l < n_lhs; l++) for (int k = mv.list_off[l]; k < mv.list_off[l + 1]; k++) if (mv.list_col[k] < 0 || mv.list_col[k] >= n) return "bad structure hint";
    for (int i = 0; i < m; i++) {
        const int a = mv.roff[i], e = mv.roff[i + 1];
        if (a == e && mv.row_lhs[i] < 0) { const double b = mv.rhs[i]; const bool ok = mv.rtype[i] == 1 ? b >= -1e-9 : (mv.rtype[i] == 0 ? b <= 1e-9 : std::fabs(b) <= 1e-9); if (!ok) return "infeasible empty row"; continue; }
        if (hinted && mv.row_block[i] >= 0) continue;
        const int L = mv.row_lhs[i];
        const int tail = a;
        bool neg = false;
        if (L >= 0) { Fam &f = fam[(size_t)L]; if (f.first < 0) { f.first = i; f.len = mv.list_off[L + 1] - mv.list_off[L]; } }
        for (int k = tail; k < e; k++) if (mv.rcoef[k] < 0.0) neg = true;
        if (mv.rtype[i] == 0 || neg) continue;
        if (mv.rhs[i] < -1e-9) return "infeasible row";
        if (L >= 0) fam[(size_t)L].rhs_min = std::min(fam[(size_t)L].rhs_min, mv.rhs[i]);
        bound_terms(tail, e, mv.rhs[i]);
    }
    for (int l = 0; l < n_lhs; l++) if (fam[(size_t)l].first >= 0 && fam[(size_t)l].rhs_min < INF) {
        const double bnd = std::floor(fam[(size_t)l].rhs_min + 1e-9);
        for (int k = mv.list_off[l]; k < mv.list_off[l + 1]; k++) { double &u = ub[mv.list_col[k]]; u = std::min(u, bnd); }
    }
    struct Run { int col0, row0, term0, nbk, nc, nr, nt, b0; };
    std::vector<Run> runs;
    if (hinted && mv.block_runs) {
        long long col_end = 0, row_end = 0;
        auto holds = [&](const int32_t *r) -> bool {
            const long long col0 = r[0], row0 = r[1], term0 = r[2], nbk = r[3], nc = r[4], nr = r[5], nt = r[6];
            if (nbk < 2 || nc < 1 || nc > NMAX_BLOCK || nr < 1 || nt < 1 || col0 < col_end || row0 < row_end) return false;
            if (col0 + nbk * nc > n || row0 + nbk * nr > m) return false;
            if (mv.roff[row0] != term0 || (long long)mv.roff[row0 + nbk * nr] != term0 + nbk * nt) return false;
            const int b0 = blk[col0];
            if (b0 < 0 || b0 + nbk > nb) return false;
            for (long long t = 0; t < nt; t++) { const long long rel = (long long)mv.rcol[term0 + t] - col0; if (rel < 0 || rel >= nc) return false; }
            for (long long q = 0; q < nc; q++) if (blk[col0 + q] != b0) return false;
            for (long long k = 0; k < nbk; k++) {
                if (bsize[b0 + k] != nc) return false;
                const int32_t gk = mv.col_group[col0 + k * nc];
                const long long rk = row0 + k * nr;
                for (long long q = 0; q < nr; q++) if (mv.row_lhs[rk + q] >= 0 || mv.row_block[rk + q] != gk) return false;
            }
            const size_t cs = (size_t)((nbk - 1) * nc), rs = (size_t)((nbk - 1) * nr), ts = (size_t)((nbk - 1) * nt);
            { const int *bp = blk.data() + col0; bool ok = true; for (size_t q = 0; q < cs; q++) ok &= bp[q + nc] == bp[q] + 1; if (!ok) return false; }
            if (memcmp(mv.kind + col0 + nc, mv.kind + col0, cs) != 0 || memcmp(mv.col_ub + col0 + nc, mv.col_ub + col0, cs * sizeof(uint32_t)) != 0) return false;
            if (memcmp(&ub[col0 + nc], &ub[col0], cs * sizeof(double)) != 0) return false;
            if (memcmp(mv.rtype + row0 + nr, mv.rtype + row0, rs) != 0 || memcmp(mv.rhs + row0 + nr, mv.rhs + row0, rs * sizeof(double)) != 0) return false;
            if (mv.row_implied && memcmp(mv.row_implied + row0 + nr, mv.row_implied + row0, rs) != 0) return false;
            if (memcmp(mv.rcoef + term0 + nt, mv.rcoef + term0, ts * sizeof(double)) != 0) return false;
            { const int *ro = mv.roff + row0; bool ok = true; for (size_t q = 0; q <= rs; q++) ok &= (long long)ro[q + nr] - ro[q] == nt; if (!ok) return false; }
            { const int *rc = mv.rcol + term0; bool ok = true; for (size_t q = 0; q < ts; q++) ok &= (long long)rc[q + nt] - rc[q] == nc; if (!ok) return false; }
            return true;
        };
        for (int q = 0; q < mv.n_block_runs; q++) {
            const int32_t *r = mv.block_runs + (size_t)7 * q;
            if (!holds(r)) continue;
            runs.push_back({r[0], r[1], r[2], r[3], r[4], r[5], r[6], blk[r[0]]});
            col_end = (long long)r[0] + (long long)r[3] * r[4]; row_end = (long long)r[1] + (long long)r[3] * r[5];
        }
    }
    if (hinted && g_check_hints) {
        std::vector<double> chk(n, INF);
        for (int j = 0; j < n; j++) if (mv.kind[j] == 1) chk[j] = 1.0;
        for (int i = 0; i < m; i++) {
            if (mv.row_block[i] < 0 || mv.rtype[i] == 0) continue;
            bool neg = false;
            for (int k = mv.roff[i]; k < mv.roff[i + 1]; k++) if (mv.rcoef[k] < 0.0) neg = true;
            if (neg) continue;
            for (int k = mv.roff[i]; k < mv.roff[i + 1]; k++) if (mv.rcoef[k] > 0.0) chk[mv.rcol[k]] = std::min(chk[mv.rcol[k]], std::floor(mv.rhs[i] / mv.rcoef[k] + 1e-9));
        }
        std::vector<double> any(chk);
        for (int i = 0; i < m; i++) {
            if (mv.row_block[i] >= 0 || mv.rtype[i] == 0) continue;
            bool neg = false;
            for (int k = mv.roff[i]; k < mv.roff[i + 1]; k++) if (mv.rcoef[k] < 0.0) neg = true;
            if (neg) continue;
            for (int k = mv.roff[i]; k < mv.roff[i + 1]; k++) if (mv.rcoef[k] > 0.0) any[mv.rcol[k]] = std::min(any[mv.rcol[k]], std::floor(mv.rhs[i] / mv.rcoef[k] + 1e-9));
            if (mv.row_lhs[i] >= 0) for (int k = mv.list_off[mv.row_lhs[i]]; k < mv.list_off[mv.row_lhs[i] + 1]; k++) any[mv.list_col[k]] = std::min(any[mv.list_col[k]], std::floor(mv.rhs[i] + 1e-9));
        }
        for (int j = 0; j < n; j++) if (mv.col_ub[j] != UINT32_MAX && chk[j] < INF && ((double)mv.col_ub[j] > chk[j] || (double)mv.col_ub[j] < any[j])) { g_hint_mismatches++; return "structure hint: col_ub differs from what the block's rows give"; }
    }
    
    HostTables &T = P.T;
    T.n_blocks = (uint32_t)nb;
    T.blk_off.assign((size_t)nb + 1, 0);
    for (int b = 0; b < nb; b++) T.blk_off[b + 1] = T.blk_off[b] + (uint32_t)bsize[b];
    T.n_cols = T.blk_off[nb];
    P.flat_of.assign(n, -1); P.model_of.assign(T.n_cols, -1); P.block_of_flat.assign(T.n_cols, -1);
    {
        std::vector<uint32_t> cur(T.blk_off.begin(), T.blk_off.end() - 1);
        for (int j = 0; j < n; j++) if (blk[j] >= 0) { const int f = (int)cur[blk[j]]++; P.flat_of[j] = f; P.model_of[f] = j; P.block_of_flat[f] = blk[j]; }
    }
    T.col_cost.assign(T.n_cols, 0.0); T.col_a.assign((size_t)T.n_cols * MMAX_BLOCK, 0.0); T.col_cap.assign(T.n_cols, 0);
    T.blk_m.assign(nb, 0); T.blk_cap.assign((size_t)nb * MMAX_BLOCK, 0.0);
    for (uint32_t f = 0; f < T.n_cols; f++) {
        const int j = P.model_of[f];
        if (c[j] < 0.0) return "negative cost";
        if (!(ub[j] <= 65535.0)) return "column bound above 65535";
        T.col_cost[f] = c[j];
        T.col_cap[f] = (int32_t)std::floor(ub[j] + 1e-9);
    }
    struct WideRow { double h; uint8_t ge; int lhs_key; int own = -1; std::vector<std::pair<int, double>> g; };
    std::vector<WideRow> wide;
    std::vector<std::vector<std::pair<int, int32_t>>> own_lists;
    struct RowMemo { int n = -1; long long g = 1; double raw[32]; double scaled[64]; };
    RowMemo row_memo[8], memo_big; unsigned memo_next = 0;
    struct Scan { int b0 = -2; bool multi = false, has_g = false, nonneg = true; int n_bcols = 0; double amax = 0.0; };
    auto scan = [&](int a, int e, Scan &sc) {
        for (int k = a; k < e; k++) {
            const int j = mv.rcol[k];
            if (mv.rcoef[k] < 0.0) sc.nonneg = false;
            sc.amax += mv.rcoef[k] * ub[j];
            if (blk[j] < 0) { sc.has_g = true; continue; }
            sc.n_bcols++;
            if (sc.b0 == -2) sc.b0 = blk[j]; else if (blk[j] != sc.b0) sc.multi = true;
        }
    };
    size_t run_i = 0; bool run_live = false;
    auto stamp_run = [&](const Run &R) {
        const uint32_t f0 = T.blk_off[R.b0];
        const size_t col_bytes = (size_t)R.nc * MMAX_BLOCK * sizeof(double);
        for (int k = 1; k < R.nbk; k++) {
            const int b = R.b0 + k;
            T.blk_m[b] = T.blk_m[R.b0];
            memcpy(&T.blk_cap[(size_t)b * MMAX_BLOCK], &T.blk_cap[(size_t)R.b0 * MMAX_BLOCK], MMAX_BLOCK * sizeof(double));
            memcpy(&T.col_a[(size_t)T.blk_off[b] * MMAX_BLOCK], &T.col_a[(size_t)f0 * MMAX_BLOCK], col_bytes);
        }
        P.n_runs++; P.run_blocks += R.nbk;
    };
    for (int i = 0; i < m; i++) {
        if (run_live && i == runs[run_i].row0 + runs[run_i].nr) {
            stamp_run(runs[run_i]);
            i = runs[run_i].row0 + runs[run_i].nbk * runs[run_i].nr;
            run_live = false; run_i++;
            if (i >= m) break;
        }
        if (!run_live && run_i < runs.size() && i == runs[run_i].row0) {
            bool fresh = true;
            for (int k = 0; k < runs[run_i].nbk && fresh; k++) if (T.blk_m[runs[run_i].b0 + k] != 0) fresh = false;
            if (fresh) run_live = true; else run_i++;
        }
        const int a = mv.roff[i], e = mv.roff[i + 1];
        if (a == e && mv.row_lhs[i] < 0) continue;
        const bool is_le = mv.rtype[i] == 1, is_ge = mv.rtype[i] == 0;
        const double rhs = mv.rhs[i];
        const int L = mv.row_lhs[i];
        Scan sc; const int tail = a;
        bool fam_row = false;
        if (L >= 0) {
            Fam &f = fam[(size_t)L];
            if (!f.scanned) {
                f.scanned = true;
                for (int k = mv.list_off[L]; k < mv.list_off[L + 1]; k++) {
                    const int j = mv.list_col[k];
                    f.amax += ub[j];
                    if (blk[j] < 0) { f.has_g = true; continue; }
                    f.n_bcols++;
                    if (f.b0 == -2) f.b0 = blk[j]; else if (blk[j] != f.b0) f.multi = true;
                }
            }
            if (!(f.multi && !f.has_g)) return "shared list that is not a wide left-hand side";
            sc.b0 = f.b0; sc.multi = true; sc.has_g = false; sc.nonneg = true; sc.n_bcols = f.n_bcols; sc.amax = f.amax;
            fam_row = true;
        }
        const int hint_b = (hinted && !fam_row && mv.row_block[i] >= 0 && mv.row_block[i] <= max_group) ? block_of_group[mv.row_block[i]] : -1;
        if (hint_b >= 0) {
            if (mv.row_implied && mv.row_implied[i]) continue;
            sc.b0 = hint_b; sc.n_bcols = e - a;
            const int32_t hb = mv.row_block[i];
            for (int k = a; k < e; k++) {
                if (mv.col_group[mv.rcol[k]] != hb) return "structure hint: a row_block row holds a column of another block";
                if (mv.rcoef[k] < 0.0) sc.nonneg = false;
                sc.amax += mv.rcoef[k] * ub[mv.rcol[k]];
            }
        } else scan(tail, e, sc);
        if (!sc.multi && !sc.has_g && sc.b0 >= 0) {
            if (mv.row_implied && mv.row_implied[i]) continue;
            if (is_le && sc.nonneg && sc.amax <= rhs * (1.0 + 1e-12) + 1e-9) continue;
            if (!is_le || !sc.nonneg || rhs < 0.0) return "block row that is not a packing row";
            const int b0 = sc.b0, r = T.blk_m[b0];
            if (r >= MMAX_BLOCK) return "block with more than 4 rows";
            const int nt = e - a;
            const RowMemo *hit = nullptr;
            for (const RowMemo &rm : row_memo) if (rm.n == nt && memcmp(rm.raw, mv.rcoef + a, (size_t)nt * sizeof(double)) == 0) { hit = &rm; break; }
            if (!hit) {
                if (nt > 64) return "block row with more than 64 terms";
                long long vi[64], g = 0;
                for (int k = 0; k < nt; k++) {
                    const double v = mv.rcoef[a + k] * GRID, rv = round_fast(v);
                    if (rv < 1.0 || std::fabs(v - rv) > 1e-6 * std::max(1.0, rv) || rv >= 4.0e15) return "block row off the ResourceAmount grid";
                    vi[k] = (long long)rv;
                    g = gcd_ll(g, vi[k]);
                }
                if (g < 1) g = 1;
                RowMemo &rm = nt <= 32 ? row_memo[memo_next++ % 8] : memo_big;
                rm.n = nt <= 32 ? nt : -1; rm.g = g;
                if (nt <= 32) memcpy(rm.raw, mv.rcoef + a, (size_t)nt * sizeof(double));
                for (int k = 0; k < nt; k++) rm.scaled[k] = (double)(vi[k] / g);
                hit = &rm;
            }
            const long long g = hit->g;
            const double capv = rhs * GRID;
            if (capv >= 4.0e15) return "block row capacity too large";
            const long long capi = (long long)std::floor(capv + 1e-6);
            for (int k = 0; k < nt; k++) T.col_a[(size_t)P.flat_of[mv.rcol[a + k]] * MMAX_BLOCK + r] += hit->scaled[k];
            T.blk_cap[(size_t)b0 * MMAX_BLOCK + r] = (double)(capi / g);
            T.blk_m[b0] = (uint8_t)(r + 1);
            continue;
        }
        if (!is_le && !is_ge) return "equality or range row across blocks";
        if (is_le && sc.nonneg && sc.amax <= rhs * (1.0 + 1e-12) + 1e-9) continue;
        if (is_ge && sc.nonneg && rhs <= 1e-12) continue;
        if (!sc.multi && sc.has_g && sc.n_bcols >= 1 && is_le && sc.nonneg) {
            if (sc.n_bcols != 1) return "conditional bound over several columns of a block";
            CapRow cr; cr.flat = -1; cr.rhs = 0.0;
            double cx = 0.0;
            for (int k = a; k < e; k++) if (blk[mv.rcol[k]] >= 0) { cr.flat = P.flat_of[mv.rcol[k]]; cx = mv.rcoef[k]; }
            if (!(cx > 0.0)) return "conditional bound with a zero coefficient";
            cr.rhs = rhs / cx;
            for (int k = a; k < e; k++) if (blk[mv.rcol[k]] < 0) cr.g.push_back({gidx[mv.rcol[k]], mv.rcoef[k] / cx});
            P.caps.push_back(std::move(cr));
            continue;
        }
        if (sc.n_bcols == 0) return "row over global columns only";
        WideRow w; w.ge = is_ge ? 1 : 0;
        const double sign = is_le ? 1.0 : -1.0;
        w.h = sign * rhs;
        if (fam_row) {
            w.lhs_key = 2 * L + (is_ge ? 1 : 0);
        } else { w.lhs_key = -1; w.own = (int)own_lists.size(); own_lists.emplace_back(); own_lists.back().reserve((size_t)(e - a)); }
        for (int k = tail; k < e; k++) {
            const int j = mv.rcol[k];
            const double v = sign * mv.rcoef[k];
            if (blk[j] < 0) { w.g.push_back({gidx[j], v}); continue; }
            if (fam_row) return "block column behind a shared list";
            const double rv = round_fast(v);
            if (std::fabs(v - rv) > 1e-7 * std::max(1.0, std::fabs(rv)) || std::fabs(rv) > 1.0e9) return "wide row with a non-integer coefficient";
            if (rv != 0.0) own_lists.back().push_back({P.flat_of[j], (int32_t)rv});
        }
        P.row_terms += (size_t)(e - a) - w.g.size() + (fam_row ? (size_t)fam[(size_t)L].len : 0);
        wide.push_back(std::move(w));
        if ((int)wide.size() > 1024) return "more than 1024 wide rows";
    }
    
    if (run_live) stamp_run(runs[run_i]);
    for (int b = 0; b < nb; b++) if (T.blk_m[b] == 0) {
        double total = 0.0;
        for (uint32_t f = T.blk_off[b]; f < T.blk_off[b + 1]; f++) { T.col_a[(size_t)f * MMAX_BLOCK] = 1.0; total += (double)T.col_cap[f]; }
        T.blk_cap[(size_t)b * MMAX_BLOCK] = total;
        T.blk_m[b] = 1;
    }
    P.K = (int)wide.size();
    if (P.K == 0) return "no wide row";
    P.h.resize(P.K); P.ge.resize(P.K); P.g_rows.assign(P.G, {});
    P.grp_of.assign(P.K, -1);
    std::vector<std::vector<std::pair<int, int32_t>>> lhs;
    std::vector<uint64_t> lhs_hash;
    std::vector<int> group_of_key((size_t)2 * n_lhs, -1);
    auto materialise = [&](int key, std::vector<std::pair<int, int32_t>> &out) {
        const int l = key >> 1;
        const int32_t sign = (key & 1) ? -1 : 1;
        const int k0 = mv.list_off[l], k1 = mv.list_off[l + 1];
        out.resize((size_t)(k1 - k0));
        std::pair<int, int32_t> *o = out.data(); const int *fo = P.flat_of.data();
        for (int k = k0; k < k1; k++) o[k - k0] = {fo[mv.list_col[k]], sign};
    };
    auto hash_of = [](const std::vector<std::pair<int, int32_t>> &l) { uint64_t h = 1469598103934665603ull; for (auto &t : l) h = (h ^ ((uint64_t)(uint32_t)t.first | ((uint64_t)(uint32_t)t.second << 32))) * 1099511628211ull; return h; };
    std::vector<std::pair<int, int32_t>> tmp;
    for (int k = 0; k < P.K; k++) {
        WideRow &w = wide[(size_t)k];
        P.h[k] = w.h; P.ge[k] = w.ge;
        for (auto &t : w.g) P.g_rows[t.first].push_back({k, t.second});
        if (w.lhs_key >= 0 && group_of_key[(size_t)w.lhs_key] >= 0) { P.grp_of[k] = group_of_key[(size_t)w.lhs_key]; continue; }
        std::vector<std::pair<int, int32_t>> *l;
        if (w.lhs_key >= 0) { materialise(w.lhs_key, tmp); l = &tmp; } else l = &own_lists[(size_t)w.own];
        const uint64_t hsh = hash_of(*l);
        int g = -1;
        for (size_t i = 0; i < lhs.size() && g < 0; i++) if (lhs_hash[i] == hsh && lhs[i] == *l) g = (int)i;
        if (g < 0) { g = (int)lhs.size(); lhs.push_back(std::move(*l)); lhs_hash.push_back(hsh); }
        if (w.lhs_key >= 0) group_of_key[(size_t)w.lhs_key] = g;
        P.grp_of[k] = g;
    }
    P.KG = (int)lhs.size();
    if (P.KG > KMAX_HOST) return "more than 128 distinct wide left-hand sides";
    
    finish_groups(P, lhs);
    
    P.base_cap = T.col_cap;
    return nullptr;
}

uint64_t digest_of(const Prob &P) {
    using hqmilp::fnv1a; using hqmilp::fnv1a_vec;
    const HostTables &T = P.T;
    uint64_t h = hqmilp::FNV_BASIS;
    const uint32_t dims[3] = {T.n_blocks, T.n_cols, T.K}; h = fnv1a(h, dims, sizeof dims);
    h = fnv1a_vec(h, T.blk_off); h = fnv1a_vec(h, T.blk_m); h = fnv1a_vec(h, T.blk_cap); h = fnv1a_vec(h, T.col_cost); h = fnv1a_vec(h, T.col_a); h = fnv1a_vec(h, T.col_cap);
    h = fnv1a_vec(h, T.col_woff); h = fnv1a_vec(h, T.w_row); h = fnv1a_vec(h, T.w_coef);
    const int dims2[3] = {P.K, P.G, P.KG}; h = fnv1a(h, dims2, sizeof dims2);
    h = fnv1a_vec(h, P.h); h = fnv1a_vec(h, P.ge); h = fnv1a_vec(h, P.grp_of); h = fnv1a_vec(h, P.g_off); h = fnv1a_vec(h, P.g_col); h = fnv1a_vec(h, P.g_coef);
    h = fnv1a_vec(h, P.gr_off); h = fnv1a_vec(h, P.gr_row); h = fnv1a_vec(h, P.gmodel); h = fnv1a_vec(h, P.gcost); h = fnv1a_vec(h, P.flat_of); h = fnv1a_vec(h, P.model_of);
    h = fnv1a_vec(h, P.block_of_flat); h = fnv1a_vec(h, P.base_cap);
    for (const CapRow &cr : P.caps) { h = fnv1a(h, &cr.flat, sizeof cr.flat); h = fnv1a(h, &cr.rhs, sizeof cr.rhs); for (auto &t : cr.g) { h = fnv1a(h, &t.first, sizeof t.first); h = fnv1a(h, &t.second, sizeof t.second); } }
    for (const auto &gr : P.g_rows) { const uint64_t nn = gr.size(); h = fnv1a(h, &nn, 8); for (auto &t : gr) { h = fnv1a(h, &t.first, sizeof t.first); h = fnv1a(h, &t.second, sizeof t.second); } }
    return h;
}

const char *build_from_model(const ModelView &mv, Prob &P, std::vector<double> &ub, std::vector<double> &c, double &cmax) {
    const char *why = flatten_model(mv, P, ub, c, cmax);
    if (!why && g_check_hints && mv.block_runs) {
        ModelView plain = mv; plain.block_runs = nullptr; plain.n_block_runs = 0;
        Prob P2; std::vector<double> ub2, c2; double cmax2 = 0.0;
        const char *why2 = flatten_model(plain, P2, ub2, c2, cmax2);
        if (why2 || digest_of(P2) != digest_of(P) || ub2 != ub || c2 != c || cmax2 != cmax) { g_hint_mismatches++; return "structure hint: a block run's tables differ from its blocks' own"; }
    }
    if (!why && mv.run_stats) *mv.run_stats += (uint64_t)P.run_blocks;
    if (!why && mv.tables_digest) *mv.tables_digest = digest_of(P);
    return why;
}

struct Polisher {
    const Prob &P; int n;
    explicit Polisher(const Prob &p, int n_) : P(p), n(n_) {}
    bool run(std::vector<double> &x, double &value) const {
        const HostTables &T = P.T; const int K = P.K, G = P.G;
        if ((int)x.size() != n) return false;
        std::vector<double> xf(T.n_cols), B(G);
        for (uint32_t f = 0; f < T.n_cols; f++) { const double v = x[P.model_of[f]], rv = round_fast(v); if (v < -1e-9 || v > (double)P.base_cap[f] + 1e-9 || std::fabs(v - rv) > 1e-9) return false; xf[f] = rv; }
        for (int g = 0; g < G; g++) { B[g] = x[P.gmodel[g]]; if (B[g] != 0.0 && B[g] != 1.0) return false; }
        std::vector<double> bact((size_t)T.n_blocks * MMAX_BLOCK, 0.0);
        for (uint32_t b = 0; b < T.n_blocks; b++) {
            double *ba = &bact[(size_t)b * MMAX_BLOCK];
            for (uint32_t f = T.blk_off[b]; f < T.blk_off[b + 1]; f++) if (xf[f] != 0.0) for (int r = 0; r < MMAX_BLOCK; r++) ba[r] += T.col_a[(size_t)f * MMAX_BLOCK + r] * xf[f];
            for (int r = 0; r < (int)T.blk_m[b]; r++) if (ba[r] > T.blk_cap[(size_t)b * MMAX_BLOCK + r]) return false;
        }
        std::vector<double> ga(P.KG, 0.0), fl(K, 0.0);
        for (int g = 0; g < P.KG; g++) for (int t = P.g_off[g]; t < P.g_off[g + 1]; t++) ga[g] += (double)P.g_coef[t] * xf[P.g_col[t]];
        for (int g = 0; g < G; g++) if (B[g] != 0.0) for (auto &t : P.g_rows[g]) fl[t.first] += t.second * B[g];
        for (int k = 0; k < K; k++) if (ga[P.grp_of[k]] + fl[k] > P.h[k] + 1e-9 * std::max(1.0, std::fabs(P.h[k]))) return false;
        std::vector<double> cap(T.n_cols);
        for (uint32_t f = 0; f < T.n_cols; f++) cap[f] = (double)P.base_cap[f];
        for (const CapRow &cr : P.caps) { double r = cr.rhs; for (auto &t : cr.g) r -= t.second * B[t.first]; const double cc = std::floor(r + 1e-9); if (xf[cr.flat] > cc) return false; cap[cr.flat] = std::min(cap[cr.flat], cc); }
        std::vector<int> order;
        std::vector<double> gslack(P.KG, INF);
        for (int k = 0; k < K; k++) { const int g = P.grp_of[k]; gslack[g] = std::min(gslack[g], P.h[k] - (ga[g] + fl[k])); }
        for (uint32_t b = 0; b < T.n_blocks; b++) {
            const double *ba = &bact[(size_t)b * MMAX_BLOCK], *bc = &T.blk_cap[(size_t)b * MMAX_BLOCK];
            const int mb = (int)T.blk_m[b];
            for (uint32_t f = T.blk_off[b]; f < T.blk_off[b + 1]; f++) {
                if (!(T.col_cost[f] > 0.0) || cap[f] - xf[f] < 1.0) continue;
                bool room = true;
                for (uint32_t e = T.col_woff[f]; e < T.col_woff[f + 1] && room; e++) { const double a = (double)T.w_coef[e]; if (a > 0.0 && gslack[T.w_row[e]] < 0.5 * a) room = false; }
                for (int r = 0; r < mb && room; r++) { const double a = T.col_a[(size_t)f * MMAX_BLOCK + r]; if (a > 0.0 && bc[r] - ba[r] < a) room = false; }
                if (room) order.push_back((int)f);
            }
        }
        std::sort(order.begin(), order.end(), [&](int p, int q) { return T.col_cost[p] > T.col_cost[q] || (T.col_cost[p] == T.col_cost[q] && P.model_of[p] < P.model_of[q]); });
        for (int f : order) {
            double step = cap[f] - xf[f];
            if (step < 1.0) continue;
            const uint32_t b = (uint32_t)P.block_of_flat[f];
            const double *ba = &bact[(size_t)b * MMAX_BLOCK];
            for (int r = 0; r < (int)T.blk_m[b] && step >= 1.0; r++) { const double a = T.col_a[(size_t)f * MMAX_BLOCK + r]; if (a > 0.0) { const double room = T.blk_cap[(size_t)b * MMAX_BLOCK + r] - ba[r]; if (room < a) { step = 0.0; break; } step = std::min(step, std::floor(room / a + 1e-9)); } }
            for (uint32_t e = T.col_woff[f]; e < T.col_woff[f + 1] && step >= 1.0; e++) {
                const double a = (double)T.w_coef[e];
                if (!(a > 0.0)) continue;
                const int g = T.w_row[e];
                for (int q = P.gr_off[g]; q < P.gr_off[g + 1]; q++) { const int k = P.gr_row[q]; const double room = P.h[k] - (ga[g] + fl[k]); if (room < 0.5 * a) { step = 0.0; break; } step = std::min(step, std::floor(room / a + 1e-9)); }
            }
            if (step < 1.0) continue;
            xf[f] += step;
            double *bw = &bact[(size_t)b * MMAX_BLOCK];
            for (int r = 0; r < MMAX_BLOCK; r++) bw[r] += T.col_a[(size_t)f * MMAX_BLOCK + r] * step;
            for (uint32_t e = T.col_woff[f]; e < T.col_woff[f + 1]; e++) ga[T.w_row[e]] += (double)T.w_coef[e] * step;
        }
        double z = 0.0;
        for (uint32_t f = 0; f < T.n_cols; f++) { x[P.model_of[f]] = xf[f]; z += T.col_cost[f] * xf[f]; }
        for (int g = 0; g < G; g++) z += P.gcost[g] * B[g];
        value = z;
        return true;
    }
};

}

Answer solve_model(const ModelView &mv, double rel_gap, double time_limit_s, double deadline_s, bool trace, Sweeper &sw, double *cost_scale) {
    const double tp0 = now_us();
    Request rq;
    rq.n = mv.n; rq.m = mv.m; rq.rel_gap = rel_gap; rq.time_limit_s = time_limit_s; rq.deadline_s = deadline_s; rq.trace = trace;
    Solver S(rq, sw);
    std::vector<double> ub, c; double cmax = 1.0;
        if (const char *why = build_from_model(mv, S.P, ub, c, cmax)) { Answer ans; ans.why = why; return ans; }
        if (cost_scale) *cost_scale = cmax;
    Polisher pol(S.P, mv.n);
    rq.polish = [&pol](std::vector<double> &x, double &value) { return pol.run(x, value); };
    return run_solver(S, tp0);
}

void flatten_for_probe(const ModelView &mv, bool trace) {
    Prob P; std::vector<double> ub, c; double cmax = 1.0;
    const char *why = build_from_model(mv, P, ub, c, cmax);
    if (trace) fprintf(stderr, "[price] flattened for the probe alone: %s\n", why ? why : "tables built");
}

void set_check_hints(bool on) { g_check_hints = on; g_hint_mismatches = 0; }
int hint_mismatches() { return g_hint_mismatches; }

Answer solve(const Request &rq, Sweeper &sw) {
    Solver S(rq, sw);
    const double tp0 = now_us();
    if (const char *why = build(rq, S.P)) { Answer ans; ans.why = why; return ans; }
    return run_solver(S, tp0);
}

}
```

hyperqueue_amd/csrc/price.h:

```cpp
#pragma once
#include <cstdint>
#include <functional>
#include <vector>

namespace hqprice {

struct HostTables {
    uint32_t n_blocks = 0, n_cols = 0, K = 0;
    std::vector<uint32_t> blk_off; std::vector<uint8_t> blk_m; std::vector<double> blk_cap;
    std::vector<double> col_cost, col_a; std::vector<int32_t> col_cap; std::vector<uint32_t> col_woff; std::vector<uint16_t> w_row; std::vector<int32_t> w_coef;
};

struct SweepTotals {
    double cx = 0, rc = 0, bnd = 0;
    uint32_t n_budget = 0, max_steps = 0;
    std::vector<long long> act;
    std::vector<double> part_cx;
    std::vector<long long> part_act;
};
constexpr int PARTS = 16;

struct RangeValues { const double *cx = nullptr, *rc = nullptr, *bnd = nullptr; const uint32_t *steps = nullptr; const long long *part_act = nullptr; };

void totals_from_blocks(uint32_t n_blocks, uint32_t K, const double *cx, const double *rc, const double *bnd, const uint32_t *steps, const long long *part_act, SweepTotals &out);

struct Sweeper {
    virtual ~Sweeper() {}
    virtual bool begin(const HostTables &t, uint32_t max_sweeps) = 0;
    virtual bool set_caps(const int32_t *col_cap) = 0;
    virtual bool set_block_caps(const double *blk_cap) = 0;
    virtual bool sweep(const double *pi, SweepTotals &out) = 0;
    virtual bool sweep_launch(const double *pi) { pending_pi.assign(pi, pi + pending_k); return true; }
    virtual bool sweep_finish(SweepTotals &out) { return sweep(pending_pi.data(), out); }
    std::vector<double> pending_pi; uint32_t pending_k = 0;
    virtual const uint16_t *patterns(uint32_t first, uint32_t count) = 0;
    virtual void end() = 0;
    virtual bool sweep_range(const double *pi, uint32_t b0, uint32_t b1, RangeValues &out) { (void)pi; (void)b0; (void)b1; (void)out; return false; }
    double guard_s = 1e300;
    bool time_up = false;
    virtual bool merges_clock() const { return false; }
    uint32_t min_cols = 256;
    uint32_t budget = 4096;
    uint32_t stat_sweeps = 0;
    double stat_sweep_us = 0;
};

struct Request {
    int n = 0, m = 0;
    const int *roff = nullptr, *rcol = nullptr; const double *rcoef = nullptr, *rlo = nullptr, *rhi = nullptr;
    const double *row_scale = nullptr; const uint8_t *row_implied = nullptr;
    const int32_t *col_group = nullptr;
    const double *c = nullptr, *ub = nullptr;
    const double *incumbent = nullptr; double incumbent_value = 0.0;
    double rel_gap = 1e-4;
    double time_limit_s = 5.0;
    double deadline_s = 1e300;
    std::function<bool(std::vector<double> &x, double &value)> polish;
    bool trace = false;
};

struct Answer {
    bool ran = false;
    double bound = 1e300;
    std::vector<double> x;
    double x_value = 0.0;
    uint32_t sweeps = 0, rounds = 0;
    const char *why = "";
    std::vector<int> block_of; std::vector<double> block_value, rcost;
};

Answer solve(const Request &rq, Sweeper &sw);

struct ModelView {
    int n = 0, m = 0;
    const double *obj = nullptr; const uint8_t *kind = nullptr;
    const uint8_t *rtype = nullptr; const double *rhs = nullptr;
    const int *roff = nullptr, *rcol = nullptr; const double *rcoef = nullptr;
    const int32_t *col_group = nullptr; const uint8_t *row_implied = nullptr;
    const int32_t *row_lhs = nullptr, *row_lhs_len = nullptr;
    const int *list_off = nullptr, *list_col = nullptr; int n_lists = 0;
    const int32_t *row_block = nullptr; const uint32_t *col_ub = nullptr;
    const int32_t *block_runs = nullptr; int n_block_runs = 0;
    uint64_t *run_stats = nullptr;
    uint64_t *tables_digest = nullptr;
};
void set_check_hints(bool on);
int hint_mismatches();
void flatten_for_probe(const ModelView &mv, bool trace);
Answer solve_model(const ModelView &mv, double rel_gap, double time_limit_s, double deadline_s, bool trace, Sweeper &sw, double *cost_scale);

struct Exchange {
    uint32_t rank = 0, world = 1;
    virtual ~Exchange() {}
    virtual bool allgather(const void *send, void *recv, size_t bytes) = 0;
    uint64_t n_calls = 0, n_bytes = 0; double us = 0;
};

struct ShardedSweeper : Sweeper {
    Sweeper &inner; Exchange &ex;
    const HostTables *T = nullptr;
    std::vector<uint32_t> rank_b0, rank_b1, rank_p0, rank_p1;
    uint32_t max_blocks = 0, max_parts = 0, max_cols = 0;
    std::vector<unsigned char> send, recv;
    std::vector<double> cx, rc, bnd; std::vector<uint32_t> steps; std::vector<long long> part_act;
    std::vector<uint16_t> pats;
    uint32_t n_sweeps = 0;
    uint32_t min_blocks = 1025;
    bool pass = false;
    ShardedSweeper(Sweeper &in, Exchange &e, uint32_t min_blocks_) : inner(in), ex(e), min_blocks(min_blocks_) { min_cols = in.min_cols; budget = in.budget; }
    bool begin(const HostTables &t, uint32_t max_sweeps) override;
    bool set_caps(const int32_t *col_cap) override { return inner.set_caps(col_cap); }
    bool set_block_caps(const double *blk_cap) override { return inner.set_block_caps(blk_cap); }
    bool sweep(const double *pi, SweepTotals &out) override;
    const uint16_t *patterns(uint32_t first, uint32_t count) override;
    void end() override { inner.end(); T = nullptr; }
    bool merges_clock() const override { return ex.world > 1; }
};

}
```

hyperqueue_amd/csrc/price.hip:

```cpp
#include <hip/hip_runtime.h>

#include <algorithm>
#include <chrono>
#include <cstdio>
#include <cstdlib>
#include <cstring>
#include <type_traits>
#include <vector>

#include "dev_wave.h"
#include "price_core.h"
#include "price_dev.h"

namespace hqprice {

static_assert(PARTS == ASLOTS, "the master's parts are the kernel's activity slots");
constexpr int ASUB = 4;

namespace {

struct SweepResult {
    double cx, rc, bnd;
    uint32_t n_budget, max_steps;
    long long act[KMAX];
    double part_cx[ASLOTS];
    long long part_act[ASLOTS * KMAX];
    uint32_t seq;
};

struct PartVal { uint32_t nbud, mx; };

struct SweepArgs {
    Tables t;
    SweepOut out;
    uint32_t budget, seq;
    uint32_t *tickets;
    long long *tact;
    PartVal *pval;
    SweepResult *res;
    uint32_t first, local;
    double *lv_cx, *lv_rc, *lv_bnd; uint32_t *lv_steps;
    double pi[KMAX];
};

__device__ __forceinline__ double ld_dev(const double *p) { return __longlong_as_double((long long)__hip_atomic_load(reinterpret_cast<const unsigned long long *>(p), __ATOMIC_RELAXED, __HIP_MEMORY_SCOPE_AGENT)); }
__device__ __forceinline__ long long ld_dev(const long long *p) { return (long long)__hip_atomic_load(reinterpret_cast<const unsigned long long *>(p), __ATOMIC_RELAXED, __HIP_MEMORY_SCOPE_AGENT); }
__device__ __forceinline__ uint32_t ld_dev(const uint32_t *p) { return __hip_atomic_load(p, __ATOMIC_RELAXED, __HIP_MEMORY_SCOPE_AGENT); }
__device__ __forceinline__ void st_dev(long long *p, long long v) { __hip_atomic_store(reinterpret_cast<unsigned long long *>(p), (unsigned long long)v, __ATOMIC_RELAXED, __HIP_MEMORY_SCOPE_AGENT); }
__device__ __forceinline__ void st_dev(uint32_t *p, uint32_t v) { __hip_atomic_store(p, v, __ATOMIC_RELAXED, __HIP_MEMORY_SCOPE_AGENT); }
__device__ __forceinline__ void st_host(double *p, double v) { __hip_atomic_store(reinterpret_cast<unsigned long long *>(p), (unsigned long long)__double_as_longlong(v), __ATOMIC_RELAXED, __HIP_MEMORY_SCOPE_SYSTEM); }
__device__ __forceinline__ void st_host(long long *p, long long v) { __hip_atomic_store(reinterpret_cast<unsigned long long *>(p), (unsigned long long)v, __ATOMIC_RELAXED, __HIP_MEMORY_SCOPE_SYSTEM); }
__device__ __forceinline__ void st_host(uint32_t *p, uint32_t v) { __hip_atomic_store(p, v, __ATOMIC_RELAXED, __HIP_MEMORY_SCOPE_SYSTEM); }
__device__ __forceinline__ void acked() { __builtin_amdgcn_fence(__ATOMIC_RELEASE, "workgroup"); }

template <class SH, int NW>
__global__ __launch_bounds__(WAVE * NW) void k_price_sweep(const SweepArgs a) {
    __shared__ SH S;
    using WV = typename std::conditional<NW == 1, hqblock::DevWave, hqblock::DevGroup<NW>>::type;
    WV wv;
    if (NW > 1 && threadIdx.x >= WAVE) { hqblock::pool_helper(wv, S); return; }
    const uint32_t lane = threadIdx.x;
    const uint32_t nb = a.t.n_blocks, K = a.t.K, per = part_size(nb), b = a.first + blockIdx.x, p = b / per;
    solve_priced_block(wv, S, a.t, a.pi, b, a.out, a.budget);
    uint64_t *prof = a.out.prof ? a.out.prof + (size_t)b * PSLOTS : nullptr;
    const uint32_t r0 = a.first, r1 = a.first + gridDim.x;
    const uint32_t pb0 = p * per > r0 ? p * per : r0, pe = p * per + per < nb ? p * per + per : nb, pb1 = pe < r1 ? pe : r1;
    acked();
    if (prof && lane == 0) prof[11] = wv.now();
    uint32_t last = 0;
    if (lane == 0) last = __hip_atomic_fetch_add(&a.tickets[1 + p], 1u, __ATOMIC_RELAXED, __HIP_MEMORY_SCOPE_AGENT) == pb1 - pb0 - 1 ? 1u : 0u;
    last = (uint32_t)__builtin_amdgcn_readfirstlane((int)last);
    if (prof && lane == 0) prof[12] = wv.now();
    if (!last) return;
    {
        long long vs[2][ASUB];
#pragma unroll
        for (int u = 0; u < 2; u++) {
            const uint32_t k = lane + (uint32_t)u * WAVE;
#pragma unroll
            for (int sub = 0; sub < ASUB; sub++) vs[u][sub] = k < K ? ld_dev(&a.out.act[((size_t)p * ASUB + sub) * K + k]) : 0;
        }
        double *scr = &S.py[0][0];
        static_assert(sizeof(S.py) >= 256 * sizeof(double), "a round of the part's c.x values is staged in the dual pool's storage");
        uint32_t nbud = 0, mx = 0;
        double s4 = 0.0;
        for (uint32_t c0 = p * per; c0 < pe; c0 += 256) {
            double v[4]; uint32_t vst[4];
#pragma unroll
            for (int u = 0; u < 4; u++) { const uint32_t q = c0 + lane + (uint32_t)u * WAVE; v[u] = (q < pe && !a.local) ? ld_dev(&a.out.blk_cx[q]) : 0.0; vst[u] = (q >= pb0 && q < pb1) ? ld_dev(&a.out.blk_steps[q]) : 0u; }
#pragma unroll
            for (int u = 0; u < 4; u++) { scr[lane + (uint32_t)u * WAVE] = v[u]; nbud += vst[u] >> 31; const uint32_t st = vst[u] & 0x7FFFFFFFu; mx = st > mx ? st : mx; }
            wv.sync();
            const uint32_t cnt = pe - c0 < 256u ? pe - c0 : 256u;
            if (lane < 4 && !a.local) for (uint32_t i = lane; i < cnt; i += 4) s4 += scr[i];
            wv.sync();
        }
#pragma unroll
        for (int off = 32; off >= 1; off >>= 1) { nbud += __shfl_xor(nbud, off, 64); const uint32_t om = __shfl_xor(mx, off, 64); mx = om > mx ? om : mx; }
        const double s1 = __shfl(s4, 1, 64), s2 = __shfl(s4, 2, 64), s3 = __shfl(s4, 3, 64);
        const double pcx = ((s4 + s1) + s2) + s3;
#pragma unroll
        for (int u = 0; u < 2; u++) {
            const uint32_t k = lane + (uint32_t)u * WAVE;
            if (k >= K) continue;
            long long v = 0;
#pragma unroll
            for (int sub = 0; sub < ASUB; sub++) { v += vs[u][sub]; st_dev(&a.out.act[((size_t)p * ASUB + sub) * K + k], 0); }
            st_host(&a.res->part_act[(size_t)p * K + k], v);
            if (v != 0 && !a.local) atomicAdd(reinterpret_cast<unsigned long long *>(&a.tact[k]), (unsigned long long)v);
        }
        if (lane == 0) {
            st_dev(&a.pval[p].nbud, nbud); st_dev(&a.pval[p].mx, mx);
            if (!a.local) st_host(&a.res->part_cx[p], pcx);
            st_dev(&a.tickets[1 + p], 0u);
        }
        __threadfence_system();
    }
    const uint32_t p_first = r0 / per, p_last = (r1 - 1) / per;
    if (lane == 0) last = __hip_atomic_fetch_add(&a.tickets[0], 1u, __ATOMIC_RELAXED, __HIP_MEMORY_SCOPE_AGENT) == p_last - p_first ? 1u : 0u;
    last = (uint32_t)__builtin_amdgcn_readfirstlane((int)last);
    if (!last) return;
    if (a.local) {
        for (uint32_t b0 = r0 + lane; b0 < r1; b0 += WAVE * 8) {
            double vcx[8], vrc[8], vbd[8]; uint32_t vst[8];
#pragma unroll
            for (int u = 0; u < 8; u++) { const uint32_t q = b0 + (uint32_t)u * WAVE; const bool in = q < r1; vcx[u] = in ? ld_dev(&a.out.blk_cx[q]) : 0.0; vrc[u] = in ? ld_dev(&a.out.blk_rc[q]) : 0.0; vbd[u] = in ? ld_dev(&a.out.blk_bnd[q]) : 0.0; vst[u] = in ? ld_dev(&a.out.blk_steps[q]) : 0u; }
#pragma unroll
            for (int u = 0; u < 8; u++) { const uint32_t q = b0 + (uint32_t)u * WAVE; if (q < r1) { st_host(&a.lv_cx[q], vcx[u]); st_host(&a.lv_rc[q], vrc[u]); st_host(&a.lv_bnd[q], vbd[u]); st_host(&a.lv_steps[q], vst[u]); } }
        }
    } else {
        const uint32_t n_parts = (nb + per - 1) / per;
        long long ta[2] = {0, 0};
#pragma unroll
        for (int u = 0; u < 2; u++) { const uint32_t k = lane + (uint32_t)u * WAVE; if (k < K) ta[u] = ld_dev(&a.tact[k]); }
        uint32_t pn = 0, pm = 0;
        if (lane < n_parts) { pn = ld_dev(&a.pval[lane].nbud); pm = ld_dev(&a.pval[lane].mx); }
        double cx = 0.0, rc = 0.0, bnd = 0.0;
        for (uint32_t b0 = lane; b0 < nb; b0 += WAVE * 8) {
            double vcx[8], vrc[8], vbd[8];
#pragma unroll
            for (int u = 0; u < 8; u++) { const uint32_t q = b0 + (uint32_t)u * WAVE; const bool in = q < nb; vcx[u] = in ? ld_dev(&a.out.blk_cx[q]) : 0.0; vrc[u] = in ? ld_dev(&a.out.blk_rc[q]) : 0.0; vbd[u] = in ? ld_dev(&a.out.blk_bnd[q]) : 0.0; }
#pragma unroll
            for (int u = 0; u < 8; u++) { if (b0 + (uint32_t)u * WAVE >= nb) break; cx += vcx[u]; rc += vrc[u]; bnd += vbd[u]; }
        }
        double *red = &S.py[0][0];
        red[lane] = cx; red[WAVE + lane] = rc; red[2 * WAVE + lane] = bnd;
#pragma unroll
        for (int off = 8; off >= 1; off >>= 1) { pn += __shfl_xor(pn, off, 64); const uint32_t om = __shfl_xor(pm, off, 64); pm = om > pm ? om : pm; }
        wv.sync();
        double tcx = 0.0, trc = 0.0, tb = 0.0;
        if (lane == 0) for (int l = 0; l < WAVE; l++) { tcx += red[l]; trc += red[WAVE + l]; tb += red[2 * WAVE + l]; }
#pragma unroll
        for (int u = 0; u < 2; u++) {
            const uint32_t k = lane + (uint32_t)u * WAVE;
            if (k >= K) continue;
            st_dev(&a.tact[k], 0);
            st_host(&a.res->act[k], ta[u]);
            for (uint32_t i = n_parts; i < (uint32_t)ASLOTS; i++) st_host(&a.res->part_act[(size_t)i * K + k], 0);
        }
        if (lane >= n_parts && lane < (uint32_t)ASLOTS) st_host(&a.res->part_cx[lane], 0.0);
        if (lane == 0) { st_host(&a.res->cx, tcx); st_host(&a.res->rc, trc); st_host(&a.res->bnd, tb); st_host(&a.res->n_budget, pn); st_host(&a.res->max_steps, pm); }
    }
    if (lane == 0) st_dev(&a.tickets[0], 0u);
    if (prof && lane == 0) prof[13] = wv.now();
    __threadfence_system();
    wv.sync();
    if (prof && lane == 0) prof[14] = wv.now();
    if (lane == 0) __hip_atomic_store(&a.res->seq, a.seq, __ATOMIC_RELEASE, __HIP_MEMORY_SCOPE_SYSTEM);
}

constexpr size_t SYNC_ACT = 128, SYNC_PACT = SYNC_ACT + (size_t)ASLOTS * ASUB * KMAX * 8, SYNC_PVAL = SYNC_PACT + (size_t)KMAX * 8, SYNC_BYTES = SYNC_PVAL + (size_t)ASLOTS * sizeof(PartVal);

constexpr int NPROF = 13;
const int PROF_FROM[NPROF] = {0, 1, 3, 4, 5, 5, 8, 9, 10, 6, 11, 12, 13};
const int PROF_TO[NPROF]   = {1, 2, 4, 5, 6, 8, 9, 10, 6, 11, 12, 13, 14};
const char *const PROF_NAME[NPROF] = {"reduced costs + compaction", "dual pool + order + greedy fills", "level lists + root bound", "walk", "results + activities", "[results: zero the sums", "pattern + sums in LDS", "atomics + cost loads", "values]",
                                      "acknowledgements before the ticket", "part ticket", "part sums + sweep ticket + totals (last block)", "system fence (last block)"};

size_t al16(size_t v) { return (v + 15) & ~(size_t)15; }
double now_us() { return std::chrono::duration<double, std::micro>(std::chrono::steady_clock::now().time_since_epoch()).count(); }

}

DeviceSweeper::~DeviceSweeper() { h_stage.release(); h_res.release(); h_pats.release(); h_pin.release(); h_blkv.release(); d_tab.release(); d_pats.release(); d_blk.release(); d_sync.release(); d_prof.release(); }

bool DeviceSweeper::begin(const HostTables &t, uint32_t max_sweeps) {
    if (t.K > (uint32_t)KMAX || t.n_blocks == 0) return false;
    if (profile && (!h_prof.ensure((size_t)t.n_blocks * PSLOTS * 8 + 64) || !d_prof.ensure((size_t)t.n_blocks * PSLOTS * 8 + 64))) return false;
    T = &t; n_sweeps = 0; cap_sweeps = max_sweeps;
    max_block_cols = 0;
    for (uint32_t b = 0; b < t.n_blocks; b++) max_block_cols = std::max(max_block_cols, t.blk_off[b + 1] - t.blk_off[b]);
    if (force_nmax) max_block_cols = (uint32_t)hqblock::NMAX;
    const size_t nw = t.w_row.size();
    o_off = 0; o_m = al16(o_off + (size_t)(t.n_blocks + 1) * 4); o_cap = al16(o_m + t.n_blocks); o_cost = al16(o_cap + (size_t)t.n_blocks * MMAX * 8);
    o_a = al16(o_cost + (size_t)t.n_cols * 8); o_ccap = al16(o_a + (size_t)t.n_cols * MMAX * 8); o_woff = al16(o_ccap + (size_t)t.n_cols * 4);
    o_wrow = al16(o_woff + (size_t)(t.n_cols + 1) * 4); o_wcoef = al16(o_wrow + nw * 2); tab_bytes = al16(o_wcoef + nw * 4);
    if (!h_stage.ensure(tab_bytes) || !d_tab.ensure(tab_bytes) || !h_res.ensure(sizeof(SweepResult) + 64)) return false;
    if (!h_pin.ensure((size_t)std::min<uint32_t>(max_sweeps, PIN_SWEEPS) * t.n_cols * 2 + 64)) return false;
    in_flight = false;
    if (!d_pats.ensure((size_t)max_sweeps * t.n_cols * 2) || !d_blk.ensure((size_t)t.n_blocks * 28 + 64) || !d_sync.ensure(SYNC_BYTES)) return false;
    unsigned char *h = h_stage.as<unsigned char>();
    memcpy(h + o_off, t.blk_off.data(), (size_t)(t.n_blocks + 1) * 4); memcpy(h + o_m, t.blk_m.data(), t.n_blocks); memcpy(h + o_cap, t.blk_cap.data(), (size_t)t.n_blocks * MMAX * 8);
    memcpy(h + o_cost, t.col_cost.data(), (size_t)t.n_cols * 8); memcpy(h + o_a, t.col_a.data(), (size_t)t.n_cols * MMAX * 8); memcpy(h + o_ccap, t.col_cap.data(), (size_t)t.n_cols * 4);
    memcpy(h + o_woff, t.col_woff.data(), (size_t)(t.n_cols + 1) * 4);
    if (nw) { memcpy(h + o_wrow, t.w_row.data(), nw * 2); memcpy(h + o_wcoef, t.w_coef.data(), nw * 4); }
    if (hipMemcpyAsync(d_tab.p, h, tab_bytes, hipMemcpyHostToDevice, stream) != hipSuccess) return false;
    if (!sync_clean) { if (hipMemsetAsync(d_sync.p, 0, SYNC_BYTES, stream) != hipSuccess) return false; }
    SweepResult *r = h_res.as<SweepResult>();
    seq = r->seq;
    return true;
}

bool DeviceSweeper::set_caps(const int32_t *col_cap) {
    if (!T) return false;
    memcpy(h_stage.as<unsigned char>() + o_ccap, col_cap, (size_t)T->n_cols * 4);
    return hipMemcpyAsync(d_tab.as<unsigned char>() + o_ccap, h_stage.as<unsigned char>() + o_ccap, (size_t)T->n_cols * 4, hipMemcpyHostToDevice, stream) == hipSuccess;
}

bool DeviceSweeper::set_block_caps(const double *blk_cap) {
    if (!T) return false;
    const size_t bytes = (size_t)T->n_blocks * MMAX * 8;
    memcpy(h_stage.as<unsigned char>() + o_cap, blk_cap, bytes);
    return hipMemcpyAsync(d_tab.as<unsigned char>() + o_cap, h_stage.as<unsigned char>() + o_cap, bytes, hipMemcpyHostToDevice, stream) == hipSuccess;
}

bool DeviceSweeper::sweep(const double *pi, SweepTotals &out) { return launch(pi, 0, T ? T->n_blocks : 0, false, &out); }

bool DeviceSweeper::sweep_range(const double *pi, uint32_t b0, uint32_t b1, RangeValues &rv) {
    if (!T || b1 > T->n_blocks || b0 > b1) return false;
    const uint32_t nb = T->n_blocks;
    if (!h_blkv.ensure((size_t)nb * 28 + 64)) return false;
    if (b1 > b0) { if (!launch(pi, b0, b1, true, nullptr)) return false; }
    else {
        if (n_sweeps >= cap_sweeps) return false;
        SweepResult *r = h_res.as<SweepResult>();
        memset(r->part_act, 0, sizeof(r->part_act));
        n_sweeps++;
    }
    unsigned char *h = h_blkv.as<unsigned char>();
    rv = RangeValues{(const double *)h, (const double *)(h + (size_t)nb * 8), (const double *)(h + (size_t)nb * 16), (const uint32_t *)(h + (size_t)nb * 24), h_res.as<SweepResult>()->part_act};
    return true;
}

bool DeviceSweeper::launch(const double *pi, uint32_t b0, uint32_t b1, bool local, SweepTotals *outp) { return launch_only(pi, b0, b1, local) && wait_done(outp); }
bool DeviceSweeper::sweep_launch(const double *pi) { return launch_only(pi, 0, T ? T->n_blocks : 0, false); }
bool DeviceSweeper::sweep_finish(SweepTotals &out) { return wait_done(&out); }

bool DeviceSweeper::launch_only(const double *pi, uint32_t b0, uint32_t b1, bool local) {
    if (!T || n_sweeps >= cap_sweeps || b1 <= b0 || in_flight) return false;
    const HostTables &t = *T;
    unsigned char *d = d_tab.as<unsigned char>();
    SweepArgs a;
    a.t = Tables{t.n_blocks, t.n_cols, t.K, (const uint32_t *)(d + o_off), (const uint8_t *)(d + o_m), (const double *)(d + o_cap), (const double *)(d + o_cost), (const double *)(d + o_a),
                 (const int32_t *)(d + o_ccap), (const uint32_t *)(d + o_woff), (const uint16_t *)(d + o_wrow), (const int32_t *)(d + o_wcoef)};
    unsigned char *blk = d_blk.as<unsigned char>();
    uint16_t *xdst = n_sweeps < PIN_SWEEPS ? h_pin.dev<uint16_t>() + (size_t)n_sweeps * t.n_cols : d_pats.as<uint16_t>() + (size_t)n_sweeps * t.n_cols;
    a.out = SweepOut{xdst, (double *)blk, (double *)(blk + (size_t)t.n_blocks * 8), (double *)(blk + (size_t)t.n_blocks * 16),
                     (long long *)(d_sync.as<unsigned char>() + SYNC_ACT), (uint32_t *)(blk + (size_t)t.n_blocks * 24), profile ? d_prof.as<uint64_t>() : nullptr, (uint32_t)ASUB, dbg};
    a.budget = budget; a.seq = ++seq; a.tickets = d_sync.as<uint32_t>(); a.tact = (long long *)(d_sync.as<unsigned char>() + SYNC_PACT); a.pval = (PartVal *)(d_sync.as<unsigned char>() + SYNC_PVAL); a.res = h_res.dev<SweepResult>();
    a.first = b0; a.local = local ? 1u : 0u;
    if (local) { unsigned char *lv = h_blkv.dev<unsigned char>(); a.lv_cx = (double *)lv; a.lv_rc = (double *)(lv + (size_t)t.n_blocks * 8); a.lv_bnd = (double *)(lv + (size_t)t.n_blocks * 16); a.lv_steps = (uint32_t *)(lv + (size_t)t.n_blocks * 24); }
    else { a.lv_cx = a.lv_rc = a.lv_bnd = nullptr; a.lv_steps = nullptr; }
    memset(a.pi, 0, sizeof(a.pi));
    memcpy(a.pi, pi, (size_t)t.K * 8);
    const double t0 = now_us();
    const uint32_t nblk = b1 - b0;
    const int nw = force_waves == 1 || force_waves == 2 ? force_waves : 4;
#define HQ_SWEEP(SH_, NW_) hipLaunchKernelGGL((k_price_sweep<SH_, NW_>), dim3(nblk), dim3(WAVE * NW_), 0, stream, a)
#define HQ_SWEEP_N(SH_) do { if (nw == 4) HQ_SWEEP(SH_, 4); else if (nw == 2) HQ_SWEEP(SH_, 2); else HQ_SWEEP(SH_, 1); } while (0)
    if (max_block_cols <= 8) HQ_SWEEP_N(hqblock::SharedN<8>);
    else if (max_block_cols <= 16) HQ_SWEEP_N(hqblock::SharedN<16>);
    else HQ_SWEEP_N(hqblock::SharedN<hqblock::NMAX>);
#undef HQ_SWEEP_N
#undef HQ_SWEEP
    if (hipGetLastError() != hipSuccess) return false;
    in_flight = true; sync_clean = false; flight_t0 = t0; flight_blocks = b1 - b0;
    return true;
}

bool DeviceSweeper::wait_done(SweepTotals *outp) {
    if (!T || !in_flight) return false;
    in_flight = false;
    const HostTables &t = *T;
    const double t0 = flight_t0;
    volatile SweepResult *r = h_res.as<SweepResult>();
    for (uint64_t spins = 0;; spins++) {
        if (__atomic_load_n(&r->seq, __ATOMIC_ACQUIRE) == seq) break;
        if ((spins & 0xFFFF) == 0xFFFF && now_us() - t0 > 2.0e6) {
            if (hipStreamSynchronize(stream) != hipSuccess) return false;
            if (__atomic_load_n(&r->seq, __ATOMIC_ACQUIRE) != seq) return false;
            break;
        }
    }
    last_kernel_us = now_us() - t0;
    sync_clean = true;
    if (profile) {
        if (hipMemcpyAsync(h_prof.p, d_prof.p, (size_t)t.n_blocks * PSLOTS * 8, hipMemcpyDeviceToHost, stream) != hipSuccess || hipStreamSynchronize(stream) != hipSuccess) return false;
        const uint64_t *pr = h_prof.as<uint64_t>();
        for (int st = 0; st < NPROF; st++) {
            const int from = PROF_FROM[st], to = PROF_TO[st];
            std::vector<double> v; v.reserve(t.n_blocks);
            for (uint32_t b = 0; b < t.n_blocks; b++) { const uint64_t t0s = pr[(size_t)b * PSLOTS + from], t1s = pr[(size_t)b * PSLOTS + to]; if (t0s && t1s >= t0s) v.push_back((double)(t1s - t0s) / 100.0); }
            if (v.empty()) continue;
            std::sort(v.begin(), v.end()); prof_med[st] += v[v.size() / 2]; prof_max[st] += v.back();
        }
        uint64_t first = ~0ull, last_done = 0, seq_at = 0;
        for (uint32_t b = 0; b < t.n_blocks; b++) { const uint64_t *q = pr + (size_t)b * PSLOTS; if (q[0] && q[0] < first) first = q[0]; if (q[6] > last_done) last_done = q[6]; if (q[14] > seq_at) seq_at = q[14]; }
        if (first != ~0ull) { prof_span += (double)(last_done - first) / 100.0; if (seq_at) prof_tail += (double)(seq_at - last_done) / 100.0; }
        double smax = 0; for (uint32_t b = 0; b < t.n_blocks; b++) smax = std::max(smax, (double)pr[(size_t)b * PSLOTS + 7]);
        prof_steps += smax; prof_n++;
    }
    total_sweeps++; total_block_solves += flight_blocks; total_us += last_kernel_us;
    n_sweeps++;
    if (!outp) return true;
    SweepTotals &out = *outp;
    out.cx = r->cx; out.rc = r->rc; out.bnd = r->bnd; out.n_budget = r->n_budget; out.max_steps = r->max_steps;
    out.act.resize(t.K);
    for (uint32_t k = 0; k < t.K; k++) out.act[k] = r->act[k];
    out.part_cx.assign(r->part_cx, r->part_cx + ASLOTS);
    out.part_act.resize((size_t)ASLOTS * t.K);
    for (size_t i = 0; i < (size_t)ASLOTS * t.K; i++) out.part_act[i] = r->part_act[i];
    return true;
}

const uint16_t *DeviceSweeper::patterns(uint32_t first, uint32_t count) {
    if (!T || first + count > n_sweeps || in_flight) return nullptr;
    const size_t nc = T->n_cols, bytes = (size_t)count * nc * 2;
    if (first + count <= PIN_SWEEPS) return h_pin.as<uint16_t>() + (size_t)first * nc;
    if (!h_pats.ensure(bytes + 64)) return nullptr;
    if (count == 0) return h_pats.as<uint16_t>();
    const uint32_t n_pin = first < PIN_SWEEPS ? PIN_SWEEPS - first : 0;
    if (n_pin) memcpy(h_pats.p, h_pin.as<uint16_t>() + (size_t)first * nc, (size_t)n_pin * nc * 2);
    if (hipMemcpyAsync(h_pats.as<uint16_t>() + (size_t)n_pin * nc, d_pats.as<uint16_t>() + (size_t)(first + n_pin) * nc, bytes - (size_t)n_pin * nc * 2, hipMemcpyDeviceToHost, stream) != hipSuccess) return nullptr;
    if (hipStreamSynchronize(stream) != hipSuccess) return nullptr;
    return h_pats.as<uint16_t>();
}

void DeviceSweeper::end() {
    if (in_flight) { hipStreamSynchronize(stream); in_flight = false; }
    if (profile && prof_n) {
        fprintf(stderr, "[price profile] %d sweeps, per block and sweep (us; median over blocks / slowest block, averaged over the sweeps):", prof_n);
        for (int st = 0; st < NPROF; st++) fprintf(stderr, "  %s %.1f / %.1f;", PROF_NAME[st], prof_med[st] / prof_n, prof_max[st] / prof_n);
        fprintf(stderr, "  first block's start -> last block's results %.1f, -> completion word stored %.1f more;", prof_span / prof_n, prof_tail / prof_n);
        fprintf(stderr, "  most search steps of a block %.0f; sweep as the host saw it %.1f us\n", prof_steps / prof_n, total_us / (double)std::max<uint64_t>(1, total_sweeps));
        for (int st = 0; st < NPROF; st++) prof_med[st] = prof_max[st] = 0; prof_steps = 0; prof_span = prof_tail = 0; prof_n = 0;
    }
    T = nullptr;
}

}
```

hyperqueue_amd/csrc/price_dev.h:

```cpp
#pragma once
#include <hip/hip_runtime.h>

#include <cstdlib>

#include "devbuf.h"
#include "price.h"

namespace hqprice {

struct DeviceSweeper : Sweeper {
    hipStream_t stream = nullptr;
    hqbuf::PinBuf h_stage, h_res, h_pats, h_pin, h_prof, h_blkv;
    static constexpr uint32_t PIN_SWEEPS = 64;
    bool sync_clean = false;
    bool in_flight = false; double flight_t0 = 0; uint32_t flight_blocks = 0;
    bool profile = getenv("HQTICK_PRICE_PROFILE") != nullptr; double prof_med[16] = {0}, prof_max[16] = {0}, prof_steps = 0, prof_span = 0, prof_tail = 0; int prof_n = 0;
    hqbuf::DevBuf d_tab, d_pats, d_blk, d_sync, d_prof;
    const HostTables *T = nullptr;
    size_t o_off = 0, o_m = 0, o_cap = 0, o_cost = 0, o_a = 0, o_ccap = 0, o_woff = 0, o_wrow = 0, o_wcoef = 0, tab_bytes = 0;
    uint32_t n_sweeps = 0, cap_sweeps = 0, seq = 0;
    uint32_t max_block_cols = 0;
    bool force_nmax = getenv("HQTICK_PRICE_NMAX") != nullptr;
    int force_waves = getenv("HQTICK_PRICE_WAVES") ? atoi(getenv("HQTICK_PRICE_WAVES")) : 0;
    uint32_t dbg = getenv("HQTICK_PRICE_DBG") ? (uint32_t)atoi(getenv("HQTICK_PRICE_DBG")) : 0u;
    double last_kernel_us = 0;
    uint64_t total_sweeps = 0, total_block_solves = 0; double total_us = 0;
    explicit DeviceSweeper(hipStream_t s) : stream(s) {}
    ~DeviceSweeper() override;
    bool begin(const HostTables &t, uint32_t max_sweeps) override;
    bool set_caps(const int32_t *col_cap) override;
    bool set_block_caps(const double *blk_cap) override;
    bool sweep(const double *pi, SweepTotals &out) override;
    bool sweep_range(const double *pi, uint32_t b0, uint32_t b1, RangeValues &out) override;
    bool launch(const double *pi, uint32_t b0, uint32_t b1, bool local, SweepTotals *out);
    bool launch_only(const double *pi, uint32_t b0, uint32_t b1, bool local);
    bool wait_done(SweepTotals *out);
    bool sweep_launch(const double *pi) override;
    bool sweep_finish(SweepTotals &out) override;
    const uint16_t *patterns(uint32_t first, uint32_t count) override;
    void end() override;
};

}
```

hyperqueue_amd/csrc/price_emul.cpp:

```cpp
#include "price_emul.h"

#include <cstring>

#include "price_core.h"

namespace hqprice {

static_assert(PARTS == ASLOTS, "the master's parts are the kernel's activity slots");

bool EmulatedSweeper::begin(const HostTables &t, uint32_t max_sweeps) {
    T = &t; caps = t.col_cap; bcaps = t.blk_cap; n_sweeps = 0; cap_sweeps = max_sweeps;
    pats.clear();
    blk_cx.assign(t.n_blocks, 0.0); blk_rc.assign(t.n_blocks, 0.0); blk_bnd.assign(t.n_blocks, 0.0); blk_steps.assign(t.n_blocks, 0);
    return t.K <= (uint32_t)KMAX && fail_at != 0;
}
bool EmulatedSweeper::set_caps(const int32_t *c) { caps.assign(c, c + T->n_cols); return true; }
bool EmulatedSweeper::set_block_caps(const double *c) { bcaps.assign(c, c + (size_t)T->n_blocks * MMAX); return true; }
bool EmulatedSweeper::sweep_range(const double *pi, uint32_t b0, uint32_t b1, RangeValues &rv) {
    if (n_sweeps >= cap_sweeps || !T || b1 > T->n_blocks || b0 > b1) return false;
    if (fail_at >= 1 && n_sweeps == (uint32_t)(fail_at - 1)) return false;
    static thread_local hqblock::Shared *S = new hqblock::Shared();
    hqblock::HostWave wv;
    const HostTables &t = *T;
    Tables tv{t.n_blocks, t.n_cols, t.K, t.blk_off.data(), t.blk_m.data(), bcaps.data(), t.col_cost.data(), t.col_a.data(), caps.data(), t.col_woff.data(), t.w_row.data(), t.w_coef.data()};
    pats.resize((size_t)(n_sweeps + 1) * t.n_cols);
    slots.assign((size_t)ASLOTS * t.K, 0);
    SweepOut so{pats.data() + (size_t)n_sweeps * t.n_cols, blk_cx.data(), blk_rc.data(), blk_bnd.data(), slots.data(), blk_steps.data(), nullptr};
    for (uint32_t b = b0; b < b1; b++) solve_priced_block(wv, *S, tv, pi, b, so, budget);
    rv = RangeValues{blk_cx.data(), blk_rc.data(), blk_bnd.data(), blk_steps.data(), slots.data()};
    n_sweeps++;
    return true;
}
bool EmulatedSweeper::sweep(const double *pi, SweepTotals &out) {
    RangeValues rv;
    if (!sweep_range(pi, 0, T ? T->n_blocks : 0, rv)) return false;
    totals_from_blocks(T->n_blocks, T->K, rv.cx, rv.rc, rv.bnd, rv.steps, rv.part_act, out);
    return true;
}
const uint16_t *EmulatedSweeper::patterns(uint32_t first, uint32_t count) { return first + count <= n_sweeps ? pats.data() + (size_t)first * T->n_cols : nullptr; }
void EmulatedSweeper::end() {}

}
```

hyperqueue_amd/csrc/price_emul.h:

```cpp
#pragma once
#include <algorithm>
#include <vector>

#include "price.h"

namespace hqprice {

struct EmulatedSweeper : Sweeper {
    const HostTables *T = nullptr;
    std::vector<int32_t> caps;
    std::vector<double> bcaps;
    std::vector<uint16_t> pats;
    std::vector<double> blk_cx, blk_rc, blk_bnd;
    std::vector<uint32_t> blk_steps;
    std::vector<long long> slots;
    uint32_t n_sweeps = 0, cap_sweeps = 0;
    int fail_at = -1;
    bool begin(const HostTables &t, uint32_t max_sweeps) override;
    bool set_caps(const int32_t *col_cap) override;
    bool set_block_caps(const double *blk_cap) override;
    bool sweep(const double *pi, SweepTotals &out) override;
    bool sweep_range(const double *pi, uint32_t b0, uint32_t b1, RangeValues &out) override;
    const uint16_t *patterns(uint32_t first, uint32_t count) override;
    void end() override;
};

}
```

include/hqtick_debug.h:

```cpp
#ifndef HQTICK_DEBUG_H
#define HQTICK_DEBUG_H
#include <stdint.h>
#include "hqtick.h"
#ifdef __cplusplus
extern "C" {
#endif
#if defined(__GNUC__)
#pragma GCC visibility push(default)
#endif

int hqtick_debug_milp_solve(int ncols, const double *obj, const uint8_t *col_kind, int nrows, const uint8_t *row_type,
                            const double *rhs, const int *row_off, const int *row_col, const double *row_coef,
                            double time_limit_s, int canonical, double *x_out, double *obj_out, int *is_optimal,
                            long *nodes_out);

int hqtick_debug_last_order(const hqtick_ctx *ctx, uint32_t *n_runs, uint32_t *n_levels, double *order_us);

int hqtick_debug_host_stages(const hqtick_config *config, const hqtick_snapshot *snapshot, const uint8_t *vflags, const uint32_t *vtmc,
                             uint32_t n_levels, const uint64_t *levels, const uint32_t *hist, hqtick_result *out);

int hqtick_debug_host_query(const hqtick_config *config, const hqtick_snapshot *snapshot, const hqtick_query_workers *fake,
                            const uint8_t *vflags, const uint32_t *vtmc, const uint8_t *fake_vflags, const uint32_t *fake_vtmc,
                            uint32_t n_levels, const uint64_t *levels, const uint32_t *hist, hqtick_query_result *out);

int hqtick_debug_milp_was_canonical(void);
void hqtick_debug_milp_last_hull(long *solves, long *nonpacking);

void hqtick_debug_map_order_u32(const uint32_t *keys, uint32_t n, uint32_t *out_pos);

int hqtick_debug_block_solve_host(uint32_t n_cols, uint32_t n_resources, const uint32_t *ent_off, const uint32_t *ent_res, const uint8_t *ent_kind,
                                  const uint64_t *ent_amount, const uint32_t *weight, const double *pool, uint32_t n_classes, const uint64_t *free_,
                                  const uint64_t *total, const uint64_t *elig, uint32_t budget, uint32_t *x, uint32_t *status, uint32_t *steps);
void hqtick_debug_set_block_emulation(int on, uint32_t budget);
void hqtick_debug_last_stage_us(double *out3);
void hqtick_debug_last_blocks(uint32_t *n_emulated, uint32_t *n_host);

int hqtick_time_kernel(hqtick_ctx *ctx, int which, int iters, double *avg_us);
int hqtick_timeline(const hqtick_ctx *ctx, double *out, int cap);
const uint64_t *hqtick_block_profile_last(const hqtick_ctx *ctx, uint32_t *n_classes);


void hqtick_debug_set_price_emulation(int on, uint32_t min_cols);
void hqtick_debug_set_price_fault(int fail_at);
void hqtick_debug_set_fast_path(int on);
void hqtick_debug_check_model_hints(int on);
int hqtick_debug_model_hint_mismatches(void);
void hqtick_debug_set_block_runs(int on);
void hqtick_debug_last_coupled_digest(uint64_t out[4]);
void hqtick_debug_corrupt_block_runs(int on);
void hqtick_debug_last_price(uint32_t *sweeps, uint32_t *rounds);
uint32_t hqtick_debug_last_mn(const uint32_t **rq, const uint32_t **off, const uint32_t **worker);
int hqtick_debug_milp_solve_priced(int ncols, const double *obj, const uint8_t *col_kind, const int32_t *col_group, int nrows, const uint8_t *row_type,
                                   const uint8_t *row_implied, const double *rhs, const int *row_off, const int *row_col, const double *row_coef,
                                   double time_limit_s, int use_sweeps, uint32_t min_cols, double *x_out, double *obj_out, int *is_optimal, double *stats_out);

struct hqwire_tables;
struct hqwire_records;
struct hqwire_output;
int hqwire_debug_encode_host(const struct hqwire_tables *tables, const struct hqwire_records *records, const struct hqwire_output *out);
int hqwire_debug_encode_host_order(const struct hqwire_tables *tables, const struct hqwire_records *records, const struct hqwire_output *out, int order);

void hqtick_debug_set_block_guard(uint32_t verify, uint32_t tick_seq, int corrupt_mode, uint32_t corrupt_class, uint32_t corrupt_fill);
void hqtick_debug_last_block_guard(uint32_t *verified, uint32_t *mismatch, uint32_t *rejected);
void hqtick_debug_set_block_memo(int on);
uint32_t hqtick_debug_last_block_memo(void);
void hqtick_debug_set_exchange(hqtick_exchange_fn fn, void *user, uint32_t rank, uint32_t world, uint32_t min_blocks, uint32_t min_classes);
uint32_t hqtick_debug_last_exchange_calls(void);
int hqtick_debug_exchange(hqtick_ctx *ctx, const void *send, void *recv, size_t bytes_per_rank);
#if defined(__GNUC__)
#pragma GCC visibility pop
#endif
#ifdef __cplusplus
}
#endif
#endif
```

Before: 67.50 million.

## Launch first zero-price sweep on block tables before wide rows are built

Adds a hook inside model flattening that uploads only the block tables and launches the first pricing sweep (all prices zero) on the device as soon as the blocks exist. The host then builds the wide rows in parallel and uploads them afterwards via begin_wide. Because the kernel ran without wide rows, the first sweep's row activities are recomputed on the host from the returned patterns. The aim is to hide the first sweep's latency behind host-side model construction, at the cost of extra staging logic, a host activity pass and a larger device buffer reservation.

After: 72.90 million, median of 6. 8.0% higher.

```diff
diff --git a/hyperqueue_amd/csrc/debug_capi.cpp b/hyperqueue_amd/csrc/debug_capi.cpp
--- a/hyperqueue_amd/csrc/debug_capi.cpp
+++ b/hyperqueue_amd/csrc/debug_capi.cpp
@@ -1,4 +1,7 @@
 #include "../../include/hqtick_debug.h"
+
+#include <algorithm>
+#include <cstring>
 
 #include "hb_order.h"
 #include "milp.h"
@@ -78,3 +81,11 @@
 extern "C" void hqtick_debug_last_coupled_digest(uint64_t out[4]) {
     out[0] = g_block_run_probe.model; out[1] = g_block_run_probe.tables; out[2] = g_block_run_probe.runs; out[3] = g_block_run_probe.covered;
 }
+extern "C" void hqtick_debug_set_early_sweep(int on) { hqprice::set_early_sweep(on); }
+extern "C" uint32_t hqtick_debug_early_sweeps(void) { return hqprice::early_sweeps(); }
+extern "C" void hqtick_debug_capture_first_cut(int on) { hqprice::capture_first_cut(on != 0); }
+extern "C" uint32_t hqtick_debug_first_cut(unsigned char *out, uint32_t cap) {
+    const std::vector<unsigned char> &b = hqprice::first_cut_bytes();
+    if (out && cap) memcpy(out, b.data(), std::min<size_t>(cap, b.size()));
+    return (uint32_t)b.size();
+}
diff --git a/hyperqueue_amd/csrc/price.cpp b/hyperqueue_amd/csrc/price.cpp
--- a/hyperqueue_amd/csrc/price.cpp
+++ b/hyperqueue_amd/csrc/price.cpp
@@ -4,6 +4,7 @@
 #include <chrono>
 #include <cmath>
 #include <cstdio>
+#include <cstdlib>
 #include <cstring>
 #include <functional>
 #include <map>
@@ -31,6 +32,7 @@
 constexpr double BP_MAX_WORK = 3.0e9;
 
 double now_us() { return std::chrono::duration<double, std::micro>(std::chrono::steady_clock::now().time_since_epoch()).count(); }
+thread_local uint32_t g_early_sweeps = 0;
 
 struct CapRow { int flat; double rhs; std::vector<std::pair<int, double>> g; };
 
@@ -272,7 +274,50 @@
     int max_sweeps = 256;
     std::vector<std::pair<uint32_t, int32_t>> node_lo, node_caps; double node_cl = 0.0; std::vector<double> node_Al; bool at_root = true;
     bool base_caps = true;
+    enum { EARLY_NONE = 0, EARLY_LAUNCHED, EARLY_REFUSED, EARLY_FAILED };
+    int early = EARLY_NONE;
+    bool early_begun = false;
+    bool host_acts = false;
+    double tp0 = 0.0;
     Solver(const Request &r, Sweeper &s) : rq(r), sw(s) {}
+
+    void prepare_sweeper() {
+        sw.stat_sweeps = 0; sw.stat_sweep_us = 0;
+        sw.guard_s = rq.deadline_s - 0.3 * rq.time_limit_s; sw.time_up = false;
+        max_sweeps = (int)std::min<size_t>(4096, std::max<size_t>(256, ((size_t)64 << 20) / ((size_t)P.T.n_cols * 2 + 1)));
+    }
+    void launch_on_blocks() {
+        prepare_sweeper();
+        const int took = sw.begin_blocks(P.T, (uint32_t)max_sweeps);
+        if (took < 0) return;
+        if (took == 0) { early = EARLY_REFUSED; return; }
+        early_begun = true;
+        const double zero = 0.0, t0 = now_us();
+        sw.pending_k = 0;
+        if (!sw.sweep_launch(&zero)) { early = EARLY_FAILED; return; }
+        sw.stat_sweep_us += now_us() - t0;
+        early = EARLY_LAUNCHED; host_acts = true; g_early_sweeps++;
+        if (rq.trace) fprintf(stderr, "[price] first sweep (prices 0) launched on the block tables at %.3f ms\n", (now_us() - tp0) / 1e3);
+    }
+    bool activities_from_patterns(uint32_t sweep, SweepTotals &tot) {
+        const HostTables &T = P.T;
+        const uint16_t *x = sw.patterns(sweep, 1);
+        if (!x) return false;
+        const size_t KG = (size_t)P.KG;
+        const uint32_t per = (T.n_blocks + PARTS - 1) / PARTS;
+        tot.act.assign(KG, 0); tot.part_act.assign((size_t)PARTS * KG, 0);
+        const uint32_t *woff = T.col_woff.data(); const uint16_t *wr = T.w_row.data(); const int32_t *wc = T.w_coef.data();
+        for (uint32_t b = 0; b < T.n_blocks; b++) {
+            long long *pa = &tot.part_act[(size_t)(b / per) * KG];
+            for (uint32_t f = T.blk_off[b]; f < T.blk_off[b + 1]; f++) {
+                const long long xv = (long long)x[f];
+                if (!xv) continue;
+                for (uint32_t e = woff[f]; e < woff[f + 1]; e++) pa[wr[e]] += (long long)wc[e] * xv;
+            }
+        }
+        for (int p = 0; p < PARTS; p++) for (size_t k = 0; k < KG; k++) tot.act[k] += tot.part_act[(size_t)p * KG + k];
+        return true;
+    }
 
     bool evaluate_launch(const std::vector<double> &pi) {
         if ((int)cuts.size() >= max_sweeps) return false;
@@ -288,8 +333,10 @@
         if ((int)cuts.size() >= max_sweeps) return -1;
         SweepTotals tot;
         const double t0 = now_us();
-        if (launched) { if (!sw.sweep_finish(tot)) { failed = true; return -1; } }
-        else {
+        if (launched) {
+            if (!sw.sweep_finish(tot)) { failed = true; return -1; }
+            if (host_acts) { host_acts = false; if (!activities_from_patterns((uint32_t)cuts.size(), tot)) { failed = true; return -1; } }
+        } else {
             std::vector<double> pig(P.KG, 0.0);
             for (int k = 0; k < P.K; k++) pig[P.grp_of[k]] += pi[k];
             if (!sw.sweep(pig.data(), tot)) { failed = true; return -1; }
@@ -862,6 +909,7 @@
 }
 
 namespace {
+thread_local bool g_capture_cut = false; thread_local std::vector<unsigned char> g_first_cut;
 Answer run_solver(Solver &S, const double tp0) {
     Answer ans;
     const Request &rq = S.rq; Sweeper &sw = S.sw;
@@ -871,14 +919,20 @@
     Prob &P = S.P;
     if (rq.trace) fprintf(stderr, "[price] %u blocks, %u block columns, %d wide rows with %d distinct left-hand sides (%zu / %zu terms), %d flags, %zu conditional bounds\n", P.T.n_blocks, P.T.n_cols, P.K, P.KG, P.row_terms, P.T.w_row.size(), P.G, P.caps.size());
     const int K = P.K, G = P.G;
-    sw.stat_sweeps = 0; sw.stat_sweep_us = 0;
-    sw.guard_s = rq.deadline_s - 0.3 * rq.time_limit_s; sw.time_up = false;
-    S.max_sweeps = (int)std::min<size_t>(4096, std::max<size_t>(256, ((size_t)64 << 20) / ((size_t)P.T.n_cols * 2 + 1)));
-    if (!sw.begin(P.T, (uint32_t)S.max_sweeps)) { ans.why = "sweeper refused the model"; return ans; }
-    struct Ender { Sweeper &s; ~Ender() { s.end(); } } ender{sw};
-    tmark("tables handed to the sweeper");
+    struct Ender { Sweeper *s; ~Ender() { if (s) s->end(); } } ender{S.early_begun ? &sw : nullptr};
     std::vector<double> pi0(K, 0.0);
-    if (!S.evaluate_launch(pi0)) { ans.why = "sweep failed"; return ans; }
+    if (S.early == Solver::EARLY_REFUSED) { ans.why = "sweeper refused the model"; return ans; }
+    if (S.early == Solver::EARLY_FAILED) { S.failed = true; ans.why = "sweep failed"; return ans; }
+    if (S.early == Solver::EARLY_LAUNCHED) {
+        if (!sw.begin_wide()) { ans.why = "sweeper refused the model"; return ans; }
+        tmark("wide tables handed to the sweeper");
+    } else {
+        S.prepare_sweeper();
+        if (!sw.begin(P.T, (uint32_t)S.max_sweeps)) { ans.why = "sweeper refused the model"; return ans; }
+        ender.s = &sw;
+        tmark("tables handed to the sweeper");
+        if (!S.evaluate_launch(pi0)) { ans.why = "sweep failed"; return ans; }
+    }
     S.pmax.assign(K, 0.0);
     {
         double cmax = 0.0; for (double c : P.T.col_cost) cmax = std::max(cmax, c);
@@ -897,6 +951,13 @@
     tmark("price caps done");
     if (S.evaluate(pi0, true) < 0) { ans.why = "sweep failed"; return ans; }
     tmark("first sweep (prices 0) done");
+    if (g_capture_cut) {
+        const Cut &c0 = S.cuts[0];
+        auto put = [](const void *p, size_t bytes) { const unsigned char *b = (const unsigned char *)p; g_first_cut.insert(g_first_cut.end(), b, b + bytes); };
+        g_first_cut.clear();
+        put(c0.act.data(), c0.act.size() * sizeof(long long)); put(c0.pact.data(), c0.pact.size() * sizeof(long long));
+        put(&c0.cx, sizeof c0.cx); put(&c0.bnd, sizeof c0.bnd); put(c0.pcx.data(), c0.pcx.size() * sizeof(double));
+    }
     S.theta_scale = std::max(S.cuts[0].bnd, 1e-9);
     ans.ran = true;
     double best_value = rq.incumbent ? rq.incumbent_value : -INF;
@@ -1186,7 +1247,12 @@
 namespace {
 
 thread_local bool g_check_hints = false; thread_local int g_hint_mismatches = 0;
-const char *flatten_model(const ModelView &mv, Prob &P, std::vector<double> &ub, std::vector<double> &c, double &cmax) {
+thread_local int g_early_sweep = -1;
+bool early_sweep_on() {
+    static const bool env_on = !(getenv("HQPRICE_EARLY_SWEEP") && atoi(getenv("HQPRICE_EARLY_SWEEP")) == 0);
+    return g_early_sweep < 0 ? env_on : g_early_sweep != 0;
+}
+const char *flatten_model(const ModelView &mv, Prob &P, std::vector<double> &ub, std::vector<double> &c, double &cmax, const std::function<void()> *after_blocks = nullptr) {
     const int n = mv.n, m = mv.m;
     if (!mv.col_group || !mv.row_lhs || !mv.row_lhs_len) return "no structure hints";
     int max_group = -1;
@@ -1471,6 +1537,7 @@
         T.blk_cap[(size_t)b * MMAX_BLOCK] = total;
         T.blk_m[b] = 1;
     }
+    if (after_blocks && *after_blocks) (*after_blocks)();
     P.K = (int)wide.size();
     if (P.K == 0) return "no wide row";
     P.h.resize(P.K); P.ge.resize(P.K); P.g_rows.assign(P.G, {});
@@ -1527,8 +1594,8 @@
     return h;
 }
 
-const char *build_from_model(const ModelView &mv, Prob &P, std::vector<double> &ub, std::vector<double> &c, double &cmax) {
-    const char *why = flatten_model(mv, P, ub, c, cmax);
+const char *build_from_model(const ModelView &mv, Prob &P, std::vector<double> &ub, std::vector<double> &c, double &cmax, const std::function<void()> *after_blocks = nullptr) {
+    const char *why = flatten_model(mv, P, ub, c, cmax, after_blocks);
     if (!why && g_check_hints && mv.block_runs) {
         ModelView plain = mv; plain.block_runs = nullptr; plain.n_block_runs = 0;
         Prob P2; std::vector<double> ub2, c2; double cmax2 = 0.0;
@@ -1610,9 +1677,15 @@
     Request rq;
     rq.n = mv.n; rq.m = mv.m; rq.rel_gap = rel_gap; rq.time_limit_s = time_limit_s; rq.deadline_s = deadline_s; rq.trace = trace;
     Solver S(rq, sw);
+    S.tp0 = tp0;
+    if (g_capture_cut) g_first_cut.clear();
     std::vector<double> ub, c; double cmax = 1.0;
-        if (const char *why = build_from_model(mv, S.P, ub, c, cmax)) { Answer ans; ans.why = why; return ans; }
-        if (cost_scale) *cost_scale = cmax;
+    const std::function<void()> hook = [&S]() { S.launch_on_blocks(); };
+    if (const char *why = build_from_model(mv, S.P, ub, c, cmax, early_sweep_on() ? &hook : nullptr)) {
+        if (S.early_begun) sw.end();
+        Answer ans; ans.why = why; return ans;
+    }
+    if (cost_scale) *cost_scale = cmax;
     Polisher pol(S.P, mv.n);
     rq.polish = [&pol](std::vector<double> &x, double &value) { return pol.run(x, value); };
     return run_solver(S, tp0);
@@ -1625,6 +1698,10 @@
 }
 
 void set_check_hints(bool on) { g_check_hints = on; g_hint_mismatches = 0; }
+void set_early_sweep(int on) { g_early_sweep = on; g_early_sweeps = 0; }
+uint32_t early_sweeps() { return g_early_sweeps; }
+void capture_first_cut(bool on) { g_capture_cut = on; g_first_cut.clear(); }
+const std::vector<unsigned char> &first_cut_bytes() { return g_first_cut; }
 int hint_mismatches() { return g_hint_mismatches; }
 
 Answer solve(const Request &rq, Sweeper &sw) {
diff --git a/hyperqueue_amd/csrc/price.h b/hyperqueue_amd/csrc/price.h
--- a/hyperqueue_amd/csrc/price.h
+++ b/hyperqueue_amd/csrc/price.h
@@ -27,6 +27,8 @@
 struct Sweeper {
     virtual ~Sweeper() {}
     virtual bool begin(const HostTables &t, uint32_t max_sweeps) = 0;
+    virtual int begin_blocks(const HostTables &t, uint32_t max_sweeps) { (void)t; (void)max_sweeps; return -1; }
+    virtual bool begin_wide() { return false; }
     virtual bool set_caps(const int32_t *col_cap) = 0;
     virtual bool set_block_caps(const double *blk_cap) = 0;
     virtual bool sweep(const double *pi, SweepTotals &out) = 0;
@@ -86,6 +88,10 @@
 };
 void set_check_hints(bool on);
 int hint_mismatches();
+void set_early_sweep(int on);
+uint32_t early_sweeps();
+void capture_first_cut(bool on);
+const std::vector<unsigned char> &first_cut_bytes();
 void flatten_for_probe(const ModelView &mv, bool trace);
 Answer solve_model(const ModelView &mv, double rel_gap, double time_limit_s, double deadline_s, bool trace, Sweeper &sw, double *cost_scale);
 
diff --git a/hyperqueue_amd/csrc/price.hip b/hyperqueue_amd/csrc/price.hip
--- a/hyperqueue_amd/csrc/price.hip
+++ b/hyperqueue_amd/csrc/price.hip
@@ -184,30 +184,84 @@
 
 DeviceSweeper::~DeviceSweeper() { h_stage.release(); h_res.release(); h_pats.release(); h_pin.release(); h_blkv.release(); d_tab.release(); d_pats.release(); d_blk.release(); d_sync.release(); d_prof.release(); }
 
-bool DeviceSweeper::begin(const HostTables &t, uint32_t max_sweeps) {
-    if (t.K > (uint32_t)KMAX || t.n_blocks == 0) return false;
+bool DeviceSweeper::size_buffers(const HostTables &t, uint32_t max_sweeps) {
     if (profile && (!h_prof.ensure((size_t)t.n_blocks * PSLOTS * 8 + 64) || !d_prof.ensure((size_t)t.n_blocks * PSLOTS * 8 + 64))) return false;
-    T = &t; n_sweeps = 0; cap_sweeps = max_sweeps;
+    T = &t; n_sweeps = 0; cap_sweeps = max_sweeps; blocks_only = false;
     max_block_cols = 0;
     for (uint32_t b = 0; b < t.n_blocks; b++) max_block_cols = std::max(max_block_cols, t.blk_off[b + 1] - t.blk_off[b]);
     if (force_nmax) max_block_cols = (uint32_t)hqblock::NMAX;
-    const size_t nw = t.w_row.size();
     o_off = 0; o_m = al16(o_off + (size_t)(t.n_blocks + 1) * 4); o_cap = al16(o_m + t.n_blocks); o_cost = al16(o_cap + (size_t)t.n_blocks * MMAX * 8);
     o_a = al16(o_cost + (size_t)t.n_cols * 8); o_ccap = al16(o_a + (size_t)t.n_cols * MMAX * 8); o_woff = al16(o_ccap + (size_t)t.n_cols * 4);
-    o_wrow = al16(o_woff + (size_t)(t.n_cols + 1) * 4); o_wcoef = al16(o_wrow + nw * 2); tab_bytes = al16(o_wcoef + nw * 4);
-    if (!h_stage.ensure(tab_bytes) || !d_tab.ensure(tab_bytes) || !h_res.ensure(sizeof(SweepResult) + 64)) return false;
+    o_wrow = al16(o_woff + (size_t)(t.n_cols + 1) * 4);
+    if (!h_res.ensure(sizeof(SweepResult) + 64)) return false;
     if (!h_pin.ensure((size_t)std::min<uint32_t>(max_sweeps, PIN_SWEEPS) * t.n_cols * 2 + 64)) return false;
     in_flight = false;
-    if (!d_pats.ensure((size_t)max_sweeps * t.n_cols * 2) || !d_blk.ensure((size_t)t.n_blocks * 28 + 64) || !d_sync.ensure(SYNC_BYTES)) return false;
+    return d_pats.ensure((size_t)max_sweeps * t.n_cols * 2) && d_blk.ensure((size_t)t.n_blocks * 28 + 64) && d_sync.ensure(SYNC_BYTES);
+}
+
+void DeviceSweeper::stage_blocks(const HostTables &t) {
     unsigned char *h = h_stage.as<unsigned char>();
     memcpy(h + o_off, t.blk_off.data(), (size_t)(t.n_blocks + 1) * 4); memcpy(h + o_m, t.blk_m.data(), t.n_blocks); memcpy(h + o_cap, t.blk_cap.data(), (size_t)t.n_blocks * MMAX * 8);
     memcpy(h + o_cost, t.col_cost.data(), (size_t)t.n_cols * 8); memcpy(h + o_a, t.col_a.data(), (size_t)t.n_cols * MMAX * 8); memcpy(h + o_ccap, t.col_cap.data(), (size_t)t.n_cols * 4);
+}
+
+bool DeviceSweeper::begin(const HostTables &t, uint32_t max_sweeps) {
+    if (t.K > (uint32_t)KMAX || t.n_blocks == 0) return false;
+    if (!size_buffers(t, max_sweeps)) return false;
+    const size_t nw = t.w_row.size();
+    wide_room = std::max(wide_room, nw);
+    o_wcoef = al16(o_wrow + nw * 2); tab_bytes = al16(o_wcoef + nw * 4);
+    if (!h_stage.ensure(tab_bytes) || !d_tab.ensure(tab_bytes)) return false;
+    unsigned char *h = h_stage.as<unsigned char>();
+    stage_blocks(t);
     memcpy(h + o_woff, t.col_woff.data(), (size_t)(t.n_cols + 1) * 4);
     if (nw) { memcpy(h + o_wrow, t.w_row.data(), nw * 2); memcpy(h + o_wcoef, t.w_coef.data(), nw * 4); }
     if (hipMemcpyAsync(d_tab.p, h, tab_bytes, hipMemcpyHostToDevice, stream) != hipSuccess) return false;
     if (!sync_clean) { if (hipMemsetAsync(d_sync.p, 0, SYNC_BYTES, stream) != hipSuccess) return false; }
     SweepResult *r = h_res.as<SweepResult>();
     seq = r->seq;
+    return true;
+}
+
+int DeviceSweeper::begin_blocks(const HostTables &t, uint32_t max_sweeps) {
+    if (t.n_blocks == 0 || !size_buffers(t, max_sweeps)) return 0;
+    const size_t room = std::max(wide_room, (size_t)t.n_cols * 4);
+    o_wcoef = o_wrow; tab_bytes = o_wrow;
+    const size_t dev_bytes = al16(al16(o_wrow + room * 2) + room * 4);
+    if (!h_stage.ensure(o_wrow + (dev_bytes - o_woff)) || !d_tab.ensure(dev_bytes)) return 0;
+    unsigned char *h = h_stage.as<unsigned char>();
+    stage_blocks(t);
+    memset(h + o_woff, 0, o_wrow - o_woff);
+    if (hipMemcpyAsync(d_tab.p, h, o_wrow, hipMemcpyHostToDevice, stream) != hipSuccess) return 0;
+    if (!sync_clean) { if (hipMemsetAsync(d_sync.p, 0, SYNC_BYTES, stream) != hipSuccess) return 0; }
+    seq = h_res.as<SweepResult>()->seq;
+    blocks_only = true;
+    return 1;
+}
+
+bool DeviceSweeper::begin_wide() {
+    if (!T || !blocks_only) return false;
+    const HostTables &t = *T;
+    if (t.K > (uint32_t)KMAX || t.col_woff.size() != (size_t)t.n_cols + 1) return false;
+    const size_t nw = t.w_row.size();
+    wide_room = std::max(wide_room, nw);
+    o_wcoef = al16(o_wrow + nw * 2); tab_bytes = al16(o_wcoef + nw * 4);
+    const size_t wide_bytes = tab_bytes - o_woff;
+    if (o_wrow + wide_bytes > h_stage.cap || tab_bytes > d_tab.cap) {
+        if (hipStreamSynchronize(stream) != hipSuccess) return false;
+        if (!h_stage.ensure(o_wrow + wide_bytes) || !d_tab.ensure(tab_bytes)) return false;
+        unsigned char *h = h_stage.as<unsigned char>();
+        stage_blocks(t);
+        memcpy(h + o_woff, t.col_woff.data(), (size_t)(t.n_cols + 1) * 4);
+        if (nw) { memcpy(h + o_wrow, t.w_row.data(), nw * 2); memcpy(h + o_wcoef, t.w_coef.data(), nw * 4); }
+        if (hipMemcpyAsync(d_tab.p, h, tab_bytes, hipMemcpyHostToDevice, stream) != hipSuccess) return false;
+    } else {
+        unsigned char *h = h_stage.as<unsigned char>() + o_wrow;
+        memcpy(h, t.col_woff.data(), (size_t)(t.n_cols + 1) * 4);
+        if (nw) { memcpy(h + (o_wrow - o_woff), t.w_row.data(), nw * 2); memcpy(h + (o_wcoef - o_woff), t.w_coef.data(), nw * 4); }
+        if (hipMemcpyAsync(d_tab.as<unsigned char>() + o_woff, h, wide_bytes, hipMemcpyHostToDevice, stream) != hipSuccess) return false;
+    }
+    blocks_only = false;
     return true;
 }
 
@@ -248,10 +302,12 @@
 
 bool DeviceSweeper::launch_only(const double *pi, uint32_t b0, uint32_t b1, bool local) {
     if (!T || n_sweeps >= cap_sweeps || b1 <= b0 || in_flight) return false;
+    if (blocks_only && (n_sweeps != 0 || local)) return false;
     const HostTables &t = *T;
+    const uint32_t K = blocks_only ? 0u : t.K;
     unsigned char *d = d_tab.as<unsigned char>();
     SweepArgs a;
-    a.t = Tables{t.n_blocks, t.n_cols, t.K, (const uint32_t *)(d + o_off), (const uint8_t *)(d + o_m), (const double *)(d + o_cap), (const double *)(d + o_cost), (const double *)(d + o_a),
+    a.t = Tables{t.n_blocks, t.n_cols, K, (const uint32_t *)(d + o_off), (const uint8_t *)(d + o_m), (const double *)(d + o_cap), (const double *)(d + o_cost), (const double *)(d + o_a),
                  (const int32_t *)(d + o_ccap), (const uint32_t *)(d + o_woff), (const uint16_t *)(d + o_wrow), (const int32_t *)(d + o_wcoef)};
     unsigned char *blk = d_blk.as<unsigned char>();
     uint16_t *xdst = n_sweeps < PIN_SWEEPS ? h_pin.dev<uint16_t>() + (size_t)n_sweeps * t.n_cols : d_pats.as<uint16_t>() + (size_t)n_sweeps * t.n_cols;
@@ -262,7 +318,7 @@
     if (local) { unsigned char *lv = h_blkv.dev<unsigned char>(); a.lv_cx = (double *)lv; a.lv_rc = (double *)(lv + (size_t)t.n_blocks * 8); a.lv_bnd = (double *)(lv + (size_t)t.n_blocks * 16); a.lv_steps = (uint32_t *)(lv + (size_t)t.n_blocks * 24); }
     else { a.lv_cx = a.lv_rc = a.lv_bnd = nullptr; a.lv_steps = nullptr; }
     memset(a.pi, 0, sizeof(a.pi));
-    memcpy(a.pi, pi, (size_t)t.K * 8);
+    if (K) memcpy(a.pi, pi, (size_t)K * 8);
     const double t0 = now_us();
     const uint32_t nblk = b1 - b0;
     const int nw = force_waves == 1 || force_waves == 2 ? force_waves : 4;
@@ -274,7 +330,7 @@
 #undef HQ_SWEEP_N
 #undef HQ_SWEEP
     if (hipGetLastError() != hipSuccess) return false;
-    in_flight = true; sync_clean = false; flight_t0 = t0; flight_blocks = b1 - b0;
+    in_flight = true; sync_clean = false; flight_t0 = t0; flight_blocks = b1 - b0; flight_k = K;
     return true;
 }
 
@@ -315,11 +371,12 @@
     if (!outp) return true;
     SweepTotals &out = *outp;
     out.cx = r->cx; out.rc = r->rc; out.bnd = r->bnd; out.n_budget = r->n_budget; out.max_steps = r->max_steps;
-    out.act.resize(t.K);
-    for (uint32_t k = 0; k < t.K; k++) out.act[k] = r->act[k];
+    const uint32_t K = flight_k;
+    out.act.resize(K);
+    for (uint32_t k = 0; k < K; k++) out.act[k] = r->act[k];
     out.part_cx.assign(r->part_cx, r->part_cx + ASLOTS);
-    out.part_act.resize((size_t)ASLOTS * t.K);
-    for (size_t i = 0; i < (size_t)ASLOTS * t.K; i++) out.part_act[i] = r->part_act[i];
+    out.part_act.resize((size_t)ASLOTS * K);
+    for (size_t i = 0; i < (size_t)ASLOTS * K; i++) out.part_act[i] = r->part_act[i];
     return true;
 }
 
@@ -345,7 +402,7 @@
         fprintf(stderr, "  most search steps of a block %.0f; sweep as the host saw it %.1f us\n", prof_steps / prof_n, total_us / (double)std::max<uint64_t>(1, total_sweeps));
         for (int st = 0; st < NPROF; st++) prof_med[st] = prof_max[st] = 0; prof_steps = 0; prof_span = prof_tail = 0; prof_n = 0;
     }
-    T = nullptr;
-}
-
-}
+    T = nullptr; blocks_only = false;
+}
+
+}
diff --git a/hyperqueue_amd/csrc/price_dev.h b/hyperqueue_amd/csrc/price_dev.h
--- a/hyperqueue_amd/csrc/price_dev.h
+++ b/hyperqueue_amd/csrc/price_dev.h
@@ -18,6 +18,9 @@
     hqbuf::DevBuf d_tab, d_pats, d_blk, d_sync, d_prof;
     const HostTables *T = nullptr;
     size_t o_off = 0, o_m = 0, o_cap = 0, o_cost = 0, o_a = 0, o_ccap = 0, o_woff = 0, o_wrow = 0, o_wcoef = 0, tab_bytes = 0;
+    bool blocks_only = false;
+    uint32_t flight_k = 0;
+    size_t wide_room = 0;
     uint32_t n_sweeps = 0, cap_sweeps = 0, seq = 0;
     uint32_t max_block_cols = 0;
     bool force_nmax = getenv("HQTICK_PRICE_NMAX") != nullptr;
@@ -28,6 +31,10 @@
     explicit DeviceSweeper(hipStream_t s) : stream(s) {}
     ~DeviceSweeper() override;
     bool begin(const HostTables &t, uint32_t max_sweeps) override;
+    int begin_blocks(const HostTables &t, uint32_t max_sweeps) override;
+    bool begin_wide() override;
+    bool size_buffers(const HostTables &t, uint32_t max_sweeps);
+    void stage_blocks(const HostTables &t);
     bool set_caps(const int32_t *col_cap) override;
     bool set_block_caps(const double *blk_cap) override;
     bool sweep(const double *pi, SweepTotals &out) override;
diff --git a/hyperqueue_amd/csrc/price_emul.cpp b/hyperqueue_amd/csrc/price_emul.cpp
--- a/hyperqueue_amd/csrc/price_emul.cpp
+++ b/hyperqueue_amd/csrc/price_emul.cpp
@@ -12,7 +12,35 @@
     T = &t; caps = t.col_cap; bcaps = t.blk_cap; n_sweeps = 0; cap_sweeps = max_sweeps;
     pats.clear();
     blk_cx.assign(t.n_blocks, 0.0); blk_rc.assign(t.n_blocks, 0.0); blk_bnd.assign(t.n_blocks, 0.0); blk_steps.assign(t.n_blocks, 0);
+    blocks_only = held_there = false;
     return t.K <= (uint32_t)KMAX && fail_at != 0;
+}
+int EmulatedSweeper::begin_blocks(const HostTables &t, uint32_t max_sweeps) {
+    T = &t; caps = t.col_cap; bcaps = t.blk_cap; n_sweeps = 0; cap_sweeps = max_sweeps;
+    pats.clear();
+    blk_cx.assign(t.n_blocks, 0.0); blk_rc.assign(t.n_blocks, 0.0); blk_bnd.assign(t.n_blocks, 0.0); blk_steps.assign(t.n_blocks, 0);
+    zero_woff.assign((size_t)t.n_cols + 1, 0);
+    blocks_only = true; held_there = false;
+    return fail_at != 0 ? 1 : 0;
+}
+bool EmulatedSweeper::begin_wide() {
+    if (!T || !blocks_only) return false;
+    blocks_only = false;
+    return T->K <= (uint32_t)KMAX && T->col_woff.size() == (size_t)T->n_cols + 1;
+}
+bool EmulatedSweeper::sweep_launch(const double *pi) {
+    if (!blocks_only) return Sweeper::sweep_launch(pi);
+    if (!T || n_sweeps != 0 || held_there) return false;
+    RangeValues rv;
+    if (!sweep_range(pi, 0, T->n_blocks, rv)) return false;
+    totals_from_blocks(T->n_blocks, 0, rv.cx, rv.rc, rv.bnd, rv.steps, rv.part_act, held);
+    held_there = true;
+    return true;
+}
+bool EmulatedSweeper::sweep_finish(SweepTotals &out) {
+    if (!held_there) return Sweeper::sweep_finish(out);
+    out = held; held_there = false;
+    return true;
 }
 bool EmulatedSweeper::set_caps(const int32_t *c) { caps.assign(c, c + T->n_cols); return true; }
 bool EmulatedSweeper::set_block_caps(const double *c) { bcaps.assign(c, c + (size_t)T->n_blocks * MMAX); return true; }
@@ -22,9 +50,10 @@
     static thread_local hqblock::Shared *S = new hqblock::Shared();
     hqblock::HostWave wv;
     const HostTables &t = *T;
-    Tables tv{t.n_blocks, t.n_cols, t.K, t.blk_off.data(), t.blk_m.data(), bcaps.data(), t.col_cost.data(), t.col_a.data(), caps.data(), t.col_woff.data(), t.w_row.data(), t.w_coef.data()};
+    const uint32_t K = blocks_only ? 0u : t.K;
+    Tables tv{t.n_blocks, t.n_cols, K, t.blk_off.data(), t.blk_m.data(), bcaps.data(), t.col_cost.data(), t.col_a.data(), caps.data(), blocks_only ? zero_woff.data() : t.col_woff.data(), t.w_row.data(), t.w_coef.data()};
     pats.resize((size_t)(n_sweeps + 1) * t.n_cols);
-    slots.assign((size_t)ASLOTS * t.K, 0);
+    slots.assign((size_t)ASLOTS * K, 0);
     SweepOut so{pats.data() + (size_t)n_sweeps * t.n_cols, blk_cx.data(), blk_rc.data(), blk_bnd.data(), slots.data(), blk_steps.data(), nullptr};
     for (uint32_t b = b0; b < b1; b++) solve_priced_block(wv, *S, tv, pi, b, so, budget);
     rv = RangeValues{blk_cx.data(), blk_rc.data(), blk_bnd.data(), blk_steps.data(), slots.data()};
diff --git a/hyperqueue_amd/csrc/price_emul.h b/hyperqueue_amd/csrc/price_emul.h
--- a/hyperqueue_amd/csrc/price_emul.h
+++ b/hyperqueue_amd/csrc/price_emul.h
@@ -16,7 +16,14 @@
     std::vector<long long> slots;
     uint32_t n_sweeps = 0, cap_sweeps = 0;
     int fail_at = -1;
+    bool blocks_only = false, held_there = false;
+    std::vector<uint32_t> zero_woff;
+    SweepTotals held;
     bool begin(const HostTables &t, uint32_t max_sweeps) override;
+    int begin_blocks(const HostTables &t, uint32_t max_sweeps) override;
+    bool begin_wide() override;
+    bool sweep_launch(const double *pi) override;
+    bool sweep_finish(SweepTotals &out) override;
     bool set_caps(const int32_t *col_cap) override;
     bool set_block_caps(const double *blk_cap) override;
     bool sweep(const double *pi, SweepTotals &out) override;
diff --git a/include/hqtick_debug.h b/include/hqtick_debug.h
--- a/include/hqtick_debug.h
+++ b/include/hqtick_debug.h
@@ -47,6 +47,10 @@
 int hqtick_debug_model_hint_mismatches(void);
 void hqtick_debug_set_block_runs(int on);
 void hqtick_debug_last_coupled_digest(uint64_t out[4]);
+void hqtick_debug_set_early_sweep(int on);
+uint32_t hqtick_debug_early_sweeps(void);
+void hqtick_debug_capture_first_cut(int on);
+uint32_t hqtick_debug_first_cut(unsigned char *out, uint32_t cap);
 void hqtick_debug_corrupt_block_runs(int on);
 void hqtick_debug_last_price(uint32_t *sweeps, uint32_t *rounds);
 uint32_t hqtick_debug_last_mn(const uint32_t **rq, const uint32_t **off, const uint32_t **worker);
```
